# wglao/Adjoint-ODE-Adaptivity

Hardware: AMD Instinct MI355X
Metric: DOF-updates/sec, 1D DG advection fwd+adjoint sweep, N=4, K=1e6 (higher is better)
Workload: dtype f64

## Files before the change

### adjoint-ode-adaptivity_amd/csrc/dg_common.h

```cpp
#pragma once
#include <hip/hip_runtime.h>

#include <cmath>
#include <cstddef>
#include <cstdint>
#include <cstdio>
#include <cstdlib>
#include <cstring>
#include <initializer_list>
#include <new>
#include <string>
#include <tuple>
#include <vector>
#include <type_traits>
#include <utility>
#include <vector>

#include "dg_advec.h"
#include "dg_chain.h"
#include "dg_shape.h"

namespace dgk {

constexpr int kBlock = 256;
static_assert(kBlock == kTileLanes, "the shape rules (dg_shape.h) count tiles of kBlock lanes");
constexpr int kMaxNP = 9;
constexpr int kArgmaxParts = 1024;

#define DG_NL_STEP_ATTR __attribute__((amdgpu_num_sgpr(80)))
constexpr int kNLAdjMinWaves = 5;


__device__ __forceinline__ void eta_update(double* __restrict__ eta, int64_t e, double acc,
                                           int mode) {
  double v = (mode & kEtaAssign) ? acc : eta[e] + acc;
  if (mode & kEtaAbs) v = fabs(v);
  eta[e] = v;
}

__host__ __device__ constexpr int64_t rec_ld(int64_t ktot) { return (ktot + 1) & ~int64_t(1); }

template <class F> struct KernargLayout;
template <class... P> struct KernargLayout<void (*)(P...)> {
  static constexpr int kParams = int(sizeof...(P));
  using Tail = std::tuple_element_t<sizeof...(P) - 1, std::tuple<P...>>;
  static constexpr int kPointers = (0 + ... + int(std::is_pointer_v<P>));
  static constexpr size_t kTailOffset = size_t(kParams - 1) * sizeof(void*);
};

template <class F, class A>
__device__ __forceinline__ const char* kernarg_tail() {
  using L = KernargLayout<F>;
  static_assert(std::is_same_v<typename L::Tail, A>, "kernel's last parameter is not A");
  static_assert(L::kPointers == L::kParams - 1, "all parameters before A must be pointers");
  static_assert(sizeof(void*) == 8 && alignof(A) == 8, "A must follow 8-byte pointers unpadded");
  static_assert(std::is_standard_layout_v<A> && std::is_trivially_copyable_v<A>,
                "offsetof needs a standard-layout argument struct");
  return (const char*)__builtin_amdgcn_kernarg_segment_ptr() + L::kTailOffset;
}

#define DG_KAS __attribute__((address_space(4)))
template <class F, class A>
__device__ __forceinline__ const DG_KAS char* kernarg_tail_k() {
  (void)kernarg_tail<F, A>();
  return (const DG_KAS char*)__builtin_amdgcn_kernarg_segment_ptr() + KernargLayout<F>::kTailOffset;
}

constexpr size_t kKernargMax = 4096;

constexpr size_t kMarkBytes = 16384;

int fail(int code, const std::string& msg);

inline bool overlap(const void* x, size_t nx, const void* y, size_t ny) {
  const uintptr_t a = reinterpret_cast<uintptr_t>(x), b = reinterpret_cast<uintptr_t>(y);
  return a < b + ny && b < a + nx;
}

struct ArgRange {
  const char* name;
  const void* ptr;
  size_t bytes;
};

inline int disjoint(std::initializer_list<ArgRange> args) {
  for (const ArgRange* i = args.begin(); i != args.end(); ++i)
    for (const ArgRange* j = i + 1; j != args.end(); ++j)
      if (i->ptr && j->ptr && i->bytes && j->bytes && overlap(i->ptr, i->bytes, j->ptr, j->bytes))
        return fail(DG_ERR_ARG, std::string(i->name) + " and " + j->name +
                                    " overlap (the byte ranges of a call's arrays must be disjoint)");
  return DG_OK;
}

#define HIP_TRY(expr)                                                              \
  do {                                                                             \
    hipError_t e_ = (expr);                                                        \
    if (e_ != hipSuccess)                                                          \
      return ::dgk::fail(DG_ERR_HIP, std::string(#expr) + ": " + hipGetErrorString(e_));  \
  } while (0)

template <int NS> struct RK;
template <> struct RK<5> {
  __host__ __device__ static constexpr double A(int s) {
    return s == 0 ? 0.0
         : s == 1 ? -567301805773.0 / 1357537059087.0
         : s == 2 ? -2404267990393.0 / 2016746695238.0
         : s == 3 ? -3550918686646.0 / 2091501179385.0
                  : -1275806237668.0 / 842570457699.0;
  }
  __host__ __device__ static constexpr double B(int s) {
    return s == 0 ? 1432997174477.0 / 9575080441755.0
         : s == 1 ? 5161836677717.0 / 13612068292357.0
         : s == 2 ? 1720146321549.0 / 2090206949498.0
         : s == 3 ? 3134564353537.0 / 4481467310338.0
                  : 2277821191437.0 / 14882151754819.0;
  }
  __host__ __device__ static constexpr double C(int s) {
    return s == 0 ? 0.0
         : s == 1 ? 1432997174477.0 / 9575080441755.0
         : s == 2 ? 2526269341429.0 / 6820363962896.0
         : s == 3 ? 2006345519317.0 / 3224310063776.0
                  : 2802321613138.0 / 2924317926251.0;
  }
};
template <> struct RK<1> {
  __host__ __device__ static constexpr double A(int) { return 0.0; }
  __host__ __device__ static constexpr double B(int) { return 1.0; }
  __host__ __device__ static constexpr double C(int) { return 0.0; }
};

template <int NP> struct OpArgs {
  double Dm[NP * NP];
  double L0[NP];
  double L1[NP];
};

template <int NP> struct EOArgs {
  static constexpr int NE = (NP + 1) / 2;
  static constexpr int NO = NP / 2;
  double Qeo[NE * NO];
  double Qoe[NO * NE];
  double le[NE];
  double lo[NO];
};

template <int NP, int NS, int MS> struct StepArgs {
  EOArgs<NP> op;
  double sc;
  double uin[MS * NS + 1];
  int64_t ktot;
  int64_t stride;
  int64_t n0;
  int32_t K;
  int32_t xcd;
  int32_t jend;
};

template <int NP, int MS> struct AdjArgs {
  EOArgs<NP> op;
  double sc;
  double uin_res[MS];
  double src[MS];
  int64_t ktot;
  int64_t stride;
  int64_t n0;
  int32_t K;
  int32_t has_eta;
  int32_t xcd;
};

template <int NP>
__device__ __forceinline__ int load_tile(const double* __restrict__ g, int64_t e0, int64_t nd,
                                         double* __restrict__ lds) {
  const int64_t d0 = e0 * NP;
  const int64_t base = d0 & ~int64_t(1);
  const int off = int(d0 - base);
  const int nvec = (kBlock * NP + off + 1) >> 1;
  const double2* __restrict__ g2 = reinterpret_cast<const double2*>(g);
  for (int v = threadIdx.x; v < nvec; v += kBlock) {
    const int64_t gd = base + 2 * int64_t(v);
    double2 val;
    if (gd >= 0 && gd + 1 < nd) {
      val = g2[gd >> 1];
    } else {
      val.x = (gd >= 0 && gd < nd) ? g[gd] : 0.0;
      val.y = (gd + 1 >= 0 && gd + 1 < nd) ? g[gd + 1] : 0.0;
    }
    *reinterpret_cast<double2*>(&lds[2 * v]) = val;
  }
  return off;
}

template <int NP, int W> struct TileGeo {
  static constexpr int LB = kBlock * W;
  static constexpr int T = LB;
  static constexpr int kVec = (T * NP + 2 + 2 * LB - 1) / (2 * LB);
  static constexpr int kTileD = T * NP + 2;
  static constexpr int kFaceD = 4 * (T + 2);
  static constexpr int kFB = (kTileD + 1) & ~1;
  static constexpr int kLds = kFB + kFaceD;
};

template <int NP, int W> struct TileRegs {
  double2 v[TileGeo<NP, W>::kVec];
  int off;
};

template <int NP, int W, bool EDGE = true>
__device__ __forceinline__ void tile_issue(const double* __restrict__ g, int64_t e0, int64_t nd,
                                           TileRegs<NP, W>& r) {
  using G = TileGeo<NP, W>;
  const int64_t d0 = e0 * NP;
  const int64_t base = d0 & ~int64_t(1);
  r.off = int(d0 - base);
  const int nvec = (G::T * NP + r.off + 1) >> 1;
  const double2* __restrict__ g2 = reinterpret_cast<const double2*>(g);
#pragma unroll
  for (int q = 0; q < G::kVec; ++q) {
    const int v = threadIdx.x + q * G::LB;
    const int64_t gd = base + 2 * int64_t(v);
    double2 val = make_double2(0.0, 0.0);
    if (v < nvec) {
      if (!EDGE || (gd >= 0 && gd + 1 < nd)) {
        val = g2[gd >> 1];
      } else {
        if (gd >= 0 && gd < nd) val.x = g[gd];
        if (gd + 1 >= 0 && gd + 1 < nd) val.y = g[gd + 1];
      }
    }
    r.v[q] = val;
  }
}

template <int NP, int W>
__device__ __forceinline__ void tile_commit(const TileRegs<NP, W>& r, double* __restrict__ lds) {
  using G = TileGeo<NP, W>;
  const int nvec = (G::T * NP + r.off + 1) >> 1;
#pragma unroll
  for (int q = 0; q < G::kVec; ++q) {
    const int v = threadIdx.x + q * G::LB;
    if (v < nvec) *reinterpret_cast<double2*>(&lds[2 * v]) = r.v[q];
  }
}

template <int LB = kBlock>
__device__ __forceinline__ void store_run(double* __restrict__ g, int64_t o0, int64_t count,
                                          const double* __restrict__ lds) {
  double2* __restrict__ g2 = reinterpret_cast<double2*>(g);
  for (int64_t v = threadIdx.x; 2 * v < count; v += LB) {
    const double2 val = *reinterpret_cast<const double2*>(&lds[2 * v]);
    const int64_t gd = o0 + 2 * v;
    if (2 * v + 1 < count) {
      g2[gd >> 1] = val;
    } else {
      g[gd] = val.x;
    }
  }
}

template <int COUNT, int LB>
__device__ __forceinline__ void store_full(double* __restrict__ g, int64_t o0,
                                           const double* __restrict__ lds) {
  static_assert(COUNT % 2 == 0, "16-byte runs");
  constexpr int NV = COUNT / 2, NQ = (NV + LB - 1) / LB;
  double2* __restrict__ g2 = reinterpret_cast<double2*>(g + o0);
#pragma unroll
  for (int q = 0; q < NQ; ++q) {
    const int v = int(threadIdx.x) + q * LB;
    if ((q + 1) * LB <= NV || v < NV) g2[v] = *reinterpret_cast<const double2*>(&lds[2 * v]);
  }
}

__device__ __forceinline__ bool edge_tile(int64_t e0, int T, int64_t ktot, int32_t K) {
  if (e0 < 0 || e0 + T > ktot) return true;
  const int64_t kl0 = int64_t(uint32_t(e0) % uint32_t(K));
  return kl0 == 0 || kl0 + T >= K;
}

struct Elem {
  int64_t e;
  int32_t kl;
  bool inrange, first, last, valid;
};

template <int H, int T, bool EDGE = true>
__device__ __forceinline__ Elem elem_info(int64_t e0, int el, int64_t ktot, int32_t K) {
  Elem E;
  E.e = e0 + el;
  if constexpr (!EDGE) {
    E.kl = int32_t(uint32_t(E.e) % uint32_t(K));
    E.inrange = true;
    E.first = E.last = false;
    E.valid = el >= H && el < T - H;
    return E;
  }
  E.inrange = (E.e >= 0 && E.e < ktot);
  E.kl = E.inrange ? int32_t(uint32_t(E.e) % uint32_t(K)) : 0;
  E.first = (E.kl == 0);
  E.last = (E.kl == K - 1);
  E.valid = E.inrange && el >= H && el < T - H;
  return E;
}

__device__ __forceinline__ int64_t tile_of(int64_t b, int64_t n, bool xcd) {
  if (!xcd || n < 16) return b;
  const int64_t q = n / 8, r = n % 8, x = b % 8, j = b / 8;
  return (x < r ? x * (q + 1) : r * (q + 1) + (x - r) * q) + j;
}


__device__ __forceinline__ void pin(double& x) { asm volatile("" : "+v"(x)); }

template <int NP>
__device__ __forceinline__ void to_eo(const double* u, double* ev, double* od) {
  constexpr int NE = EOArgs<NP>::NE, NO = EOArgs<NP>::NO, N = NP - 1;
#pragma unroll
  for (int k = 0; k < NO; ++k) {
    ev[k] = 0.5 * (u[k] + u[N - k]);
    od[k] = 0.5 * (u[k] - u[N - k]);
  }
  if constexpr (NE > NO) ev[NO] = u[NO];
}

template <int NP>
__device__ __forceinline__ void from_eo(const double* ev, const double* od, double* u) {
  constexpr int NE = EOArgs<NP>::NE, NO = EOArgs<NP>::NO, N = NP - 1;
#pragma unroll
  for (int k = 0; k < NO; ++k) {
    u[k] = ev[k] + od[k];
    u[N - k] = ev[k] - od[k];
  }
  if constexpr (NE > NO) u[NO] = ev[NO];
}

template <int NP, int W, int H>
__device__ __forceinline__ void stage_out(double* __restrict__ lds, const double (*ev)[(NP + 1) / 2],
                                          const double (*od)[NP / 2], bool dual) {
  constexpr int T = TileGeo<NP, W>::T, EPL = 1;
  constexpr int NE = EOArgs<NP>::NE, NO = EOArgs<NP>::NO, N = NP - 1;
  const int lane = threadIdx.x;
#pragma unroll
  for (int m = 0; m < EPL; ++m) {
    const int el = m * T + lane;
    if (el >= H && el < T - H) {
      double* o = lds + (el - H) * NP;
      if (dual) {
#pragma unroll
        for (int k = 0; k < NO; ++k) {
          o[k] = 0.5 * (ev[m][k] + od[m][k]);
          o[N - k] = 0.5 * (ev[m][k] - od[m][k]);
        }
        if constexpr (NE > NO) o[NO] = ev[m][NO];
      } else {
        from_eo<NP>(ev[m], od[m], o);
      }
    }
  }
}

}

struct dg_plan : dgk::Shape {
  int N = 0;
  int64_t K = 0, batch = 0;
  int64_t K_cap = 0;
  double a = 0.0;
  int inflow = 0, scheme = 0;
  double s_uniform = 0.0;
  double r[dgk::kMaxNP], V[dgk::kMaxNP * dgk::kMaxNP], invV[dgk::kMaxNP * dgk::kMaxNP],
      Dr[dgk::kMaxNP * dgk::kMaxNP],
      LIFT[dgk::kMaxNP * 2];
  double* d_scale = nullptr;
  double* d_VX = nullptr;
  double* d_scratch = nullptr;
  double* d_scratch2 = nullptr;
  double* d_pv = nullptr;
  int64_t* d_pi = nullptr;
  void* d_mark = nullptr;
  void* d_sweep = nullptr;
  int32_t* d_nl_list = nullptr;
  int64_t nl_list_tiles = 0, nl_list_steps = 0;
  size_t sweep_bytes = 0;
  size_t sweep_sync = 0;
  int64_t sweep_items = -1;
  uint64_t sweep_sig = 0;
  std::vector<void*> sweep_retired;
  uint32_t* h_sweep_err = nullptr;
  uint32_t* d_sweep_err = nullptr;
  uint64_t* sweep_trace = nullptr;
  int cu_count = 0;
  int flux = 0;
  int limiter = 0;
  double tvb_M = 0.0;
  bool nonlinear() const { return flux != 0 || limiter != 0; }
};

namespace dgk {

inline double inflow_value(const dg_plan* p, double t) {
  if (p->inflow == DG_INFLOW_ZERO) return 0.0;
  return (p->inflow == DG_INFLOW_SIN_A2T) ? -std::sin(p->a * p->a * t) : -std::sin(p->a * t);
}

template <int NP> OpArgs<NP> make_op(const dg_plan* p, double scale = 1.0) {
  OpArgs<NP> op;
  for (int i = 0; i < NP; ++i) {
    for (int j = 0; j < NP; ++j) op.Dm[i * NP + j] = scale * (-p->a * p->Dr[i * NP + j]);
    op.L0[i] = scale * ((-p->a / 2.0) * p->LIFT[i * 2 + 0]);
    op.L1[i] = scale * ((p->a / 2.0) * p->LIFT[i * 2 + 1]);
  }
  return op;
}

template <int NP> bool make_eo(const dg_plan* p, double scale, EOArgs<NP>* out, bool fold = false) {
  constexpr int NE = EOArgs<NP>::NE, NO = EOArgs<NP>::NO, N = NP - 1;
  double Dm[NP][NP], L0[NP], L1[NP], T[NP][NP] = {}, Ti[NP][NP] = {};
  for (int i = 0; i < NP; ++i) {
    for (int j = 0; j < NP; ++j) Dm[i][j] = scale * (-p->a * p->Dr[i * NP + j]);
    L0[i] = scale * ((-p->a / 2.0) * p->LIFT[i * 2 + 0]);
    L1[i] = scale * ((p->a / 2.0) * p->LIFT[i * 2 + 1]);
  }
  for (int k = 0; k < NO; ++k) {
    T[k][k] += 0.5; T[k][N - k] += 0.5;
    T[NE + k][k] += 0.5; T[NE + k][N - k] -= 0.5;
    Ti[k][k] += 1.0; Ti[k][NE + k] += 1.0;
    Ti[N - k][k] += 1.0; Ti[N - k][NE + k] -= 1.0;
  }
  if (NE > NO) { T[NO][NO] = 1.0; Ti[NO][NO] = 1.0; }
  double TD[NP][NP], Q[NP][NP], l0[NP], l1[NP];
  for (int i = 0; i < NP; ++i)
    for (int j = 0; j < NP; ++j) {
      double t = 0.0;
      for (int k = 0; k < NP; ++k) t += T[i][k] * Dm[k][j];
      TD[i][j] = t;
    }
  double qmax = 0.0, lmax = 0.0;
  for (int i = 0; i < NP; ++i) {
    for (int j = 0; j < NP; ++j) {
      double t = 0.0;
      for (int k = 0; k < NP; ++k) t += TD[i][k] * Ti[k][j];
      Q[i][j] = t;
      qmax = std::fmax(qmax, std::fabs(t));
    }
    double a0 = 0.0, a1 = 0.0;
    for (int k = 0; k < NP; ++k) {
      a0 += T[i][k] * L0[k];
      a1 += T[i][k] * L1[k];
    }
    l0[i] = a0;
    l1[i] = a1;
    lmax = std::fmax(lmax, std::fmax(std::fabs(a0), std::fabs(a1)));
  }
  bool ok = true;
  const double tq = 1e-12 * qmax, tl = 1e-12 * lmax;
  for (int i = 0; i < NE; ++i)
    for (int j = 0; j < NE; ++j) ok = ok && std::fabs(Q[i][j]) <= tq;
  for (int i = 0; i < NO; ++i)
    for (int j = 0; j < NO; ++j) ok = ok && std::fabs(Q[NE + i][NE + j]) <= tq;
  for (int k = 0; k < NE; ++k) ok = ok && std::fabs(l0[k] + l1[k]) <= tl;
  for (int k = 0; k < NO; ++k) ok = ok && std::fabs(l0[NE + k] - l1[NE + k]) <= tl;
  if (out) {
    for (int k = 0; k < NE; ++k)
      for (int j = 0; j < NO; ++j) out->Qeo[k * NO + j] = Q[k][NE + j];
    for (int k = 0; k < NO; ++k)
      for (int j = 0; j < NE; ++j) out->Qoe[k * NE + j] = Q[NE + k][j];
    for (int k = 0; k < NE; ++k) out->le[k] = 0.5 * (l0[k] - l1[k]);
    for (int k = 0; k < NO; ++k) out->lo[k] = 0.5 * (l0[NE + k] + l1[NE + k]);
    if (fold) {
      for (int k = 0; k < NE; ++k) out->Qeo[k * NO] += 2.0 * out->le[k];
      for (int k = 0; k < NO; ++k) out->Qoe[k * NE] += 2.0 * out->lo[k];
    }
  }
  return ok;
}

template <int MAXNP = kMaxNP, class F> int dispatch_np(int np, F&& f) {
  static_assert(MAXNP >= 2 && MAXNP <= kMaxNP, "Np range");
  switch (np) {
    case 2: return f(std::integral_constant<int, 2>{});
    case 3: if constexpr (MAXNP >= 3) return f(std::integral_constant<int, 3>{}); break;
    case 4: if constexpr (MAXNP >= 4) return f(std::integral_constant<int, 4>{}); break;
    case 5: if constexpr (MAXNP >= 5) return f(std::integral_constant<int, 5>{}); break;
    case 6: if constexpr (MAXNP >= 6) return f(std::integral_constant<int, 6>{}); break;
    case 7: if constexpr (MAXNP >= 7) return f(std::integral_constant<int, 7>{}); break;
    case 8: if constexpr (MAXNP >= 8) return f(std::integral_constant<int, 8>{}); break;
    case 9: if constexpr (MAXNP >= 9) return f(std::integral_constant<int, 9>{}); break;
    default: break;
  }
  return fail(DG_ERR_ARG, "unsupported Np (2 .. " + std::to_string(MAXNP) + ")");
}
int nl_rhs(const dg_plan* p, const double* u, double* rhs, double t, hipStream_t st);
int nl_query(const dg_plan* p, int64_t out[3]);
int nl_fwd(dg_plan* p, double* u, double t0, double dt, int nsteps, double* snapshots,
           uint16_t* decisions, hipStream_t st);
int nl_adj(dg_plan* p, double* w, const double* snapshots, double t0, double dt, int nsteps,
           double src_coef, double* eta, int flags, const uint16_t* decisions, hipStream_t st);

int axpy_copy(const double* w, const double* u, double c, double* out, int64_t n, hipStream_t st);

inline auto field_copy(int64_t field, hipStream_t st) {
  return [=](double* dst, const double* src) -> int {
    HIP_TRY(hipMemcpyAsync(dst, src, sizeof(double) * field, hipMemcpyDeviceToDevice, st));
    return DG_OK;
  };
}

int fwd_march(const dg_plan* p, FwdShape s, double* u, const double* tn, double dt, int nsteps,
              double* snapshots, hipStream_t st);

int wave_launch_step(const dg_plan* p, int ms, const double* in, double* snap, double* last,
                     const double* times, double dt, hipStream_t st);

struct SweepBufs {
  double* U[9];
  double* W[9];
  double* rec;
  double* eta;
  double* part;
  uint32_t* sync;
  int64_t* am_idx;
  double* am_val;
  int64_t* am_nf;
  double* am_pv;
  int64_t* am_pi;
  uint32_t* err_host;
  int32_t spin_limit;
};
int sweep_waves_per_simd(const dg_plan* p, int waves);
int sweep_launch_rec(dg_plan* p, int waves, int msf, int msa, const SweepBufs& b, double t0,
                     double dt, int nsteps, int mode, hipStream_t st);
int sweep_sync_words();
int sweep_scratch(dg_plan* p, size_t sync_bytes, size_t data_bytes, hipStream_t st, char** data);
int sweep_watchdog(dg_plan* p);
int sweep_err_word();

int pair_launch_step_rec(const dg_plan* p, int ms, const double* in, double* rec, double* last,
                         const double* times, double dt, hipStream_t st, int64_t n0, bool jend);
int pair_launch_step_snap(const dg_plan* p, int ms, const double* in, double* snap,
                          const double* times, double dt, hipStream_t st);
int pair_launch_adj_rec(const dg_plan* p, int ms, const double* win, double* wout,
                        const double* rec, double* eta, int em, const double* t_next, double dt,
                        hipStream_t st, int64_t n0);

}
```

### adjoint-ode-adaptivity_amd/csrc/dg_ovl_tiles.h

```cpp
#pragma once
#include "dg_rec_tiles.h"

namespace dgr {

constexpr int kOvGL = kOvG / 2;

template <int NP, int NW> struct OvGeo {
  static constexpr int LB = 64 * NW;
  static constexpr int T = NW * kOvS + 2 * kOvG;
  static constexpr int kTileD = T * NP + 2;
  static constexpr int kVec = (kTileD + 2 * LB - 1) / (2 * LB);
  static constexpr int kXSlot = 2 * NP;
  static constexpr int kXBuf = NW * 2 * kOvGL * kXSlot;
  static constexpr int kXD = 2 * kXBuf;
  static constexpr int kLds = ((kTileD > kXD ? kTileD : kXD) + 1) & ~1;
  static_assert(kOvS % 2 == 0 && T % 2 == 0, "lane pairs at even elements");
};

__device__ __forceinline__ double ov_shr1(double x) {
  const long long b = __double_as_longlong(x);
  const int lo = int(b), hi = int(b >> 32);
  const int rl = __builtin_amdgcn_update_dpp(lo, lo, 0x138, 0xf, 0xf, false);
  const int rh = __builtin_amdgcn_update_dpp(hi, hi, 0x138, 0xf, 0xf, false);
  return __hiloint2double(rh, rl);
}
__device__ __forceinline__ double ov_shl1(double x) {
  const long long b = __double_as_longlong(x);
  const int lo = int(b), hi = int(b >> 32);
  const int rl = __builtin_amdgcn_update_dpp(lo, lo, 0x130, 0xf, 0xf, false);
  const int rh = __builtin_amdgcn_update_dpp(hi, hi, 0x130, 0xf, 0xf, false);
  return __hiloint2double(rh, rl);
}

struct OvLane {
  int wv, j, el0;
  bool own;
};
__device__ __forceinline__ OvLane ov_lane() {
  OvLane L;
  const int lane = threadIdx.x;
  L.wv = lane >> 6;
  L.j = lane & 63;
  L.el0 = L.wv * kOvS + 2 * L.j;
  L.own = L.j >= kOvGL && L.j < 64 - kOvGL;
  return L;
}

template <int NP, int NW>
__device__ __forceinline__ void ov_exchange(double* __restrict__ xb, const OvLane& L,
                                            double (*se)[(NP + 1) / 2], double (*so)[NP / 2]) {
  constexpr int NE = EOArgs<NP>::NE, NO = EOArgs<NP>::NO, SL = 2 * NP;
  static_assert(SL % 2 == 0, "16-byte slots");
  int slot = -1;
  if (L.j >= kOvGL && L.j < 2 * kOvGL) slot = (L.wv * 2 + 0) * kOvGL + (L.j - kOvGL);
  else if (L.j >= 64 - 2 * kOvGL && L.j < 64 - kOvGL)
    slot = (L.wv * 2 + 1) * kOvGL + (L.j - (64 - 2 * kOvGL));
  if (slot >= 0) {
    double v[SL];
#pragma unroll
    for (int m = 0; m < 2; ++m) {
#pragma unroll
      for (int k = 0; k < NE; ++k) v[m * NP + k] = se[m][k];
#pragma unroll
      for (int k = 0; k < NO; ++k) v[m * NP + NE + k] = so[m][k];
    }
    double2* p = reinterpret_cast<double2*>(xb + slot * SL);
#pragma unroll
    for (int q = 0; q < NP; ++q) p[q] = double2{v[2 * q], v[2 * q + 1]};
  }
  __syncthreads();
  int src = -1;
  if (L.j < kOvGL) {
    if (L.wv > 0) src = ((L.wv - 1) * 2 + 1) * kOvGL + L.j;
  } else if (L.j >= 64 - kOvGL) {
    if (L.wv < NW - 1) src = ((L.wv + 1) * 2 + 0) * kOvGL + (L.j - (64 - kOvGL));
  }
  if (src >= 0) {
    double v[SL];
    const double2* p = reinterpret_cast<const double2*>(xb + src * SL);
#pragma unroll
    for (int q = 0; q < NP; ++q) {
      const double2 t = p[q];
      v[2 * q] = t.x;
      v[2 * q + 1] = t.y;
    }
#pragma unroll
    for (int m = 0; m < 2; ++m) {
#pragma unroll
      for (int k = 0; k < NE; ++k) se[m][k] = v[m * NP + k];
#pragma unroll
      for (int k = 0; k < NO; ++k) so[m][k] = v[m * NP + NE + k];
    }
  }
}

template <int NP, int NW, int H, bool EDGE, bool WT>
__device__ __forceinline__ void ov_store(double* __restrict__ g, int64_t o0, int64_t nd,
                                         double* __restrict__ lds, const OvLane& L,
                                         const double (*ev)[(NP + 1) / 2],
                                         const double (*od)[NP / 2], bool dual) {
  using G = OvGeo<NP, NW>;
  constexpr int T = G::T, TE = T - 2 * H;
  constexpr int NE = EOArgs<NP>::NE, NO = EOArgs<NP>::NO, N = NP - 1;
  if (L.own) {
#pragma unroll
    for (int m = 0; m < 2; ++m) {
      const int el = L.el0 + m;
      if (el >= H && el < T - H) {
        double* o = lds + (el - H) * NP;
        if (dual) {
#pragma unroll
          for (int k = 0; k < NO; ++k) {
            o[k] = 0.5 * (ev[m][k] + od[m][k]);
            o[N - k] = 0.5 * (ev[m][k] - od[m][k]);
          }
          if constexpr (NE > NO) o[NO] = ev[m][NO];
        } else {
          from_eo<NP>(ev[m], od[m], o);
        }
      }
    }
  }
  __syncthreads();
  const int64_t rem = nd - o0;
  if constexpr (EDGE) {
    if constexpr (WT) store_run_wt<G::LB>(g, o0, rem < int64_t(TE) * NP ? rem : int64_t(TE) * NP, lds);
    else store_run<G::LB>(g, o0, rem < int64_t(TE) * NP ? rem : int64_t(TE) * NP, lds);
  } else {
    if constexpr (WT) store_full_wt<TE * NP, G::LB>(g, o0, lds);
    else store_full<TE * NP, G::LB>(g, o0, lds);
  }
}

template <int NP, bool UNI, int NW, int MS, bool EDGE, bool WT>
__device__ __forceinline__ void ov_step_tile(double* __restrict__ lds, int64_t tile,
                                             const double* __restrict__ uin,
                                             double* __restrict__ rec, double* __restrict__ last,
                                             const double* __restrict__ scale,
                                             const RpOp<NP>& c, OpSrc<NP> os,
                                             const double* kb, int64_t n0, bool jend) {
  using G = OvGeo<NP, NW>;
  constexpr int T = G::T, E = 2;
  constexpr int H = RpHalo<MS>::F;
  constexpr int TE = T - 2 * H;
  static_assert(TE % 2 == 0 && TE > 0 && H % 2 == 0 && H >= kOvG, "overlapped tiles");
  constexpr int NE = EOArgs<NP>::NE, NO = EOArgs<NP>::NO;
  constexpr int CB = G::kLds;
  constexpr int CR = CB + MS * 5;
  const int lane = threadIdx.x;
  const OvLane L = ov_lane();
  const int64_t e0 = tile * TE - H;
  const int64_t ec = e0 > 0 ? e0 : 0;
  const int64_t nd = c.ktot * NP;

  const int off = tile_load<G, NP, EDGE, WT>(uin, e0, nd, lds);
  if constexpr (EDGE) {
    if (lane <= MS * 6) lds[CB + lane] = kb[lane];
  }
  __syncthreads();
  double ue[E][NE], uo[E][NO];
  Elem El[E];
  double sc[E], jv[E];
#pragma unroll
  for (int m = 0; m < E; ++m) {
    const int el = L.el0 + m;
    const double* us = lds + off + el * NP;
    to_eo<NP>(us, ue[m], uo[m]);
    El[m] = elem_info<H, T, EDGE>(e0, el, c.ktot, c.K);
    El[m].valid = El[m].valid && L.own;
    sc[m] = c.sc;
    if constexpr (!UNI) sc[m] *= El[m].inrange ? scale[El[m].kl] : 0.0;
    jv[m] = us[0] - ((EDGE && El[m].first) ? lds[CR] : us[-1]);
  }
  if (n0 >= 1) rp_rec_put<E, EDGE, WT>(rec, n0 - 1, c.ktot, El, jv, ec);
  __syncthreads();

  const double b4 = c.beta[4], b5 = c.beta[5], b3 = c.beta[3], b2 = c.beta[2];
  double te[E][NE], to[E][NO];
#pragma unroll 1
  for (int st = 0; st < MS; ++st) {
#pragma unroll
    for (int l = 0; l < 5; ++l) {
      double v0[E], vN[E];
#pragma unroll
      for (int m = 0; m < E; ++m) {
        const double e = (l == 0) ? ue[m][0] : te[m][0], o = (l == 0) ? uo[m][0] : to[m][0];
        v0[m] = e + o;
        vN[m] = e - o;
      }
      const double fromL = ov_shr1(vN[E - 1]), fromR = ov_shl1(v0[0]);
      double pe[E][NE], po[E][NO];
      {
        const auto& op = os.get();
#pragma unroll
        for (int m = 0; m < E; ++m) {
#pragma unroll
          for (int k = 0; k < NE; ++k) {
            const double* vo = (l == 0) ? uo[m] : to[m];
            double a;
            int j0 = 0;
            if (UNI && l >= 3) {
              a = ue[m][k];
            } else if (UNI && l >= 1) {
              a = (l == 1 ? b3 : b2) * ue[m][k];
            } else {
              a = op.Qeo[k * NO] * vo[0];
              j0 = 1;
            }
#pragma unroll
            for (int j = j0; j < NO; ++j) a = fma(op.Qeo[k * NO + j], vo[j], a);
            pe[m][k] = a;
          }
#pragma unroll
          for (int k = 0; k < NO; ++k) {
            const double* ve = (l == 0) ? ue[m] : te[m];
            double a;
            int j0 = 0;
            if (UNI && l >= 3) {
              a = uo[m][k];
            } else if (UNI && l >= 1) {
              a = (l == 1 ? b3 : b2) * uo[m][k];
            } else {
              a = op.Qoe[k * NE] * ve[0];
              j0 = 1;
            }
#pragma unroll
            for (int j = j0; j < NE; ++j) a = fma(op.Qoe[k * NE + j], ve[j], a);
            po[m][k] = a;
          }
        }
      }
#pragma unroll
      for (int m = 0; m < E; ++m) {
#pragma unroll
        for (int k = 0; k < NE; ++k) pin(pe[m][k]);
#pragma unroll
        for (int k = 0; k < NO; ++k) pin(po[m][k]);
      }
      double bnd = 0.0, urec = 0.0;
      if constexpr (EDGE) {
        bnd = lds[CB + st * 5 + l];
        if (l == 0) urec = lds[CR + st];
      }
      const auto& ol = os.get();
#pragma unroll
      for (int m = 0; m < E; ++m) {
        double vL = (m == 0) ? fromL : vN[m - 1];
        double vR = (m == E - 1) ? fromR : v0[m + 1];
        if (l == 0) jv[m] = v0[m] - ((EDGE && El[m].first) ? urec : vL);
        if constexpr (EDGE) {
          vL = El[m].first ? bnd : vL;
          vR = El[m].last ? vN[m] : vR;
        }
        const double dlt = vR - vL, sig = -(vL + vR);
#pragma unroll
        for (int k = 0; k < NE; ++k) {
          const double z = fma(ol.le[k], dlt, pe[m][k]);
          if constexpr (UNI) {
            if (l == 0) te[m][k] = fma(b5, z, b4 * ue[m][k]);
            else if (l < 4) te[m][k] = z;
            else ue[m][k] = z;
          } else {
            if (l == 0) te[m][k] = fma(b5 * sc[m], z, b4 * ue[m][k]);
            else if (l < 3) te[m][k] = fma(sc[m], z, (l == 1 ? b3 : b2) * ue[m][k]);
            else if (l == 3) te[m][k] = fma(sc[m], z, ue[m][k]);
            else ue[m][k] = fma(sc[m], z, ue[m][k]);
          }
        }
#pragma unroll
        for (int k = 0; k < NO; ++k) {
          const double z = fma(ol.lo[k], sig, po[m][k]);
          if constexpr (UNI) {
            if (l == 0) to[m][k] = fma(b5, z, b4 * uo[m][k]);
            else if (l < 4) to[m][k] = z;
            else uo[m][k] = z;
          } else {
            if (l == 0) to[m][k] = fma(b5 * sc[m], z, b4 * uo[m][k]);
            else if (l < 3) to[m][k] = fma(sc[m], z, (l == 1 ? b3 : b2) * uo[m][k]);
            else if (l == 3) to[m][k] = fma(sc[m], z, uo[m][k]);
            else uo[m][k] = fma(sc[m], z, uo[m][k]);
          }
        }
      }
      if (l == 0 && st >= 1) rp_rec_put<E, EDGE, WT>(rec, n0 + st - 1, c.ktot, El, jv, ec);
    }
    if (st < MS - 1 || jend) ov_exchange<NP, NW>(lds + (st & 1) * G::kXBuf, L, ue, uo);
  }
  if (jend) {
    double u0[E], uN[E];
#pragma unroll
    for (int m = 0; m < E; ++m) {
      u0[m] = ue[m][0] + uo[m][0];
      uN[m] = ue[m][0] - uo[m][0];
    }
    const double fromL = ov_shr1(uN[E - 1]);
#pragma unroll
    for (int m = 0; m < E; ++m) {
      double uL = (m == 0) ? fromL : uN[m - 1];
      if constexpr (EDGE) uL = El[m].first ? lds[CR + MS] : uL;
      jv[m] = u0[m] - uL;
    }
    rp_rec_put<E, EDGE, WT>(rec, n0 + MS - 1, c.ktot, El, jv, ec);
  }
  __syncthreads();
  ov_store<NP, NW, H, EDGE, WT>(last, tile * TE * NP, nd, lds, L, ue, uo, false);
}

template <int NP, bool UNI, int NW, int MS, bool EDGE, bool WT>
__device__ __forceinline__ void ov_adj_tile(double* __restrict__ lds, int64_t tile,
                                            const double* __restrict__ win,
                                            double* __restrict__ wout,
                                            const double* __restrict__ rec,
                                            EtaSink& es,
                                            const double* __restrict__ scale,
                                            const RpOp<NP>& c, OpSrc<NP> os, int64_t n0) {
  using G = OvGeo<NP, NW>;
  constexpr int T = G::T, E = 2;
  constexpr int H = RpHalo<MS>::A;
  constexpr int TE = T - 2 * H;
  static_assert(TE % 2 == 0 && TE > 0 && H % 2 == 0 && H >= kOvG, "overlapped tiles");
  constexpr int NE = EOArgs<NP>::NE, NO = EOArgs<NP>::NO, N = NP - 1;
  const OvLane L = ov_lane();
  const int64_t e0 = tile * TE - H;
  const int64_t ec = e0 > 0 ? e0 : 0;
  const int64_t nd = c.ktot * NP;
  const int64_t ea = e0 + L.el0;
  const int has_eta = es.mode;

  const int off = tile_load<G, NP, EDGE, WT>(win, e0, nd, lds);
  double jn[E + 1];
  rp_rec_get<E, EDGE, WT>(rec, n0 + MS - 1, c.ktot, ea, ec, jn);
  __syncthreads();
  double we[E][NE], wo[E][NO];
  Elem El[E];
  double sc[E], eacc[E];
#pragma unroll
  for (int m = 0; m < E; ++m) {
    const int el = L.el0 + m;
    const double* w = lds + off + el * NP;
#pragma unroll
    for (int k = 0; k < NO; ++k) {
      we[m][k] = w[k] + w[N - k];
      wo[m][k] = w[k] - w[N - k];
    }
    if constexpr (NE > NO) we[m][NO] = w[NO];
    El[m] = elem_info<H, T, EDGE>(e0, el, c.ktot, c.K);
    El[m].valid = El[m].valid && L.own;
    sc[m] = c.sc;
    if constexpr (!UNI) sc[m] *= El[m].inrange ? scale[El[m].kl] : 0.0;
    eacc[m] = 0.0;
  }
  __syncthreads();

  const double b4 = c.beta[4], b5 = c.beta[5], b3 = c.beta[3], b2 = c.beta[2];
  double te[E][NE], to[E][NO];
#pragma unroll 1
  for (int st = MS - 1; st >= 0; --st) {
    double jc[E + 1];
#pragma unroll
    for (int m = 0; m <= E; ++m) jc[m] = jn[m];
    if (has_eta) {
      const auto& op = os.get();
#pragma unroll
      for (int m = 0; m < E; ++m) {
        double pe = 0.0, po = 0.0;
#pragma unroll
        for (int k = 0; k < NE; ++k) pe = fma(op.le[k], we[m][k], pe);
#pragma unroll
        for (int k = 0; k < NO; ++k) po = fma(op.lo[k], wo[m][k], po);
        const bool lst = EDGE && El[m].last;
        const double dd = lst ? jc[m] : jc[m] + jc[m + 1];
        const double ds = lst ? jc[m] : jc[m] - jc[m + 1];
        double cc = fma(dd, pe, ds * po);
        if constexpr (!UNI) cc *= sc[m];
        eacc[m] += cc;
      }
    }
    if (st > 0) rp_rec_get<E, EDGE, WT>(rec, n0 + st - 1, c.ktot, ea, ec, jn);
#pragma unroll
    for (int l = 0; l < 5; ++l) {
      double g0[E], g1[E], qe[E][NE], qo[E][NO];
      const auto& ol = os.get();
#pragma unroll
      for (int m = 0; m < E; ++m) {
        double gd = 0.0, gs = 0.0;
#pragma unroll
        for (int k = 0; k < NE; ++k) {
          const double v = (l == 0) ? we[m][k] : te[m][k];
          qe[m][k] = UNI ? v : sc[m] * v;
          gd = fma(ol.le[k], qe[m][k], gd);
        }
#pragma unroll
        for (int k = 0; k < NO; ++k) {
          const double v = (l == 0) ? wo[m][k] : to[m][k];
          qo[m][k] = UNI ? v : sc[m] * v;
          gs = fma(ol.lo[k], qo[m][k], gs);
        }
        g0[m] = gd + gs;
        g1[m] = gs - gd;
      }
      const double fromL = ov_shr1(g1[E - 1]), fromR = ov_shl1(g0[0]);
      double ae[E][NE], ao[E][NO];
      const auto& oq = os.get();
#pragma unroll
      for (int m = 0; m < E; ++m) {
#pragma unroll
        for (int j = 0; j < NO; ++j) {
          double t;
          int k0 = 0;
          if (l >= 3) {
            t = wo[m][j];
          } else if (l >= 1) {
            t = (l == 1 ? b3 : b2) * wo[m][j];
          } else {
            t = oq.Qeo[j] * qe[m][0];
            k0 = 1;
          }
#pragma unroll
          for (int k = k0; k < NE; ++k) t = fma(oq.Qeo[k * NO + j], qe[m][k], t);
          ao[m][j] = t;
        }
#pragma unroll
        for (int j = 0; j < NE; ++j) {
          double t;
          int k0 = 0;
          if (l >= 3) {
            t = we[m][j];
          } else if (l >= 1) {
            t = (l == 1 ? b3 : b2) * we[m][j];
          } else {
            t = oq.Qoe[j] * qo[m][0];
            k0 = 1;
          }
#pragma unroll
          for (int k = k0; k < NO; ++k) t = fma(oq.Qoe[k * NE + j], qo[m][k], t);
          ae[m][j] = t;
        }
#pragma unroll
        for (int k = 0; k < NO; ++k) pin(ao[m][k]);
#pragma unroll
        for (int k = 0; k < NE; ++k) pin(ae[m][k]);
      }
#pragma unroll
      for (int m = 0; m < E; ++m) {
        double gl = (m == 0) ? fromL : g1[m - 1];
        double gr = (m == E - 1) ? fromR : g0[m + 1];
        if constexpr (EDGE) {
          gl = El[m].first ? 0.0 : gl;
          gr = El[m].last ? g1[m] : gr;
        }
        ae[m][0] -= gl + gr;
        ao[m][0] += gr - gl;
#pragma unroll
        for (int k = 0; k < NE; ++k) {
          if (l == 0) te[m][k] = fma(b5, ae[m][k], b4 * we[m][k]);
          else if (l < 4) te[m][k] = ae[m][k];
          else we[m][k] = ae[m][k];
        }
#pragma unroll
        for (int k = 0; k < NO; ++k) {
          if (l == 0) to[m][k] = fma(b5, ao[m][k], b4 * wo[m][k]);
          else if (l < 4) to[m][k] = ao[m][k];
          else wo[m][k] = ao[m][k];
        }
      }
    }
    if (st > 0) ov_exchange<NP, NW>(lds + ((MS - 1 - st) & 1) * G::kXBuf, L, we, wo);
  }
  if (has_eta) {
    if constexpr (WT) {
      const __amdgpu_buffer_rsrc_t ro = wt_rsrc(es.part_out ? es.part_out + ec : es.eta + ec);
#pragma unroll
      for (int m = 0; m < E; ++m) {
        if (!El[m].valid) continue;
        const uint32_t o = uint32_t(El[m].e - ec) * 8u;
        if (es.part_out) {
          wt_st8(ro, o, eacc[m]);
        } else {
          double v;
          if (es.nparts > 0) {
            v = wt_ld8(wt_rsrc(es.part_in + ec), o);
            if (!(has_eta & kEtaAssign)) v = es.eta[El[m].e] + v;
            for (int q = 1; q < es.nparts; ++q)
              v = v + wt_ld8(wt_rsrc(es.part_in + q * es.part_ld + ec), o);
            v = v + eacc[m];
          } else {
            v = (has_eta & kEtaAssign) ? eacc[m] : es.eta[El[m].e] + eacc[m];
          }
          if (has_eta & kEtaAbs) v = fabs(v);
          wt_st8(ro, o, v);
          if (es.argmax && am_better(fabs(v), El[m].e, es.bv, es.bi)) {
            es.bv = fabs(v);
            es.bi = El[m].e;
          }
        }
      }
    } else {
#pragma unroll
      for (int m = 0; m < E; ++m)
        if (El[m].valid) eta_update(es.eta, El[m].e, eacc[m], has_eta);
    }
  }
  __syncthreads();
  ov_store<NP, NW, H, EDGE, WT>(wout, tile * TE * NP, nd, lds, L, we, wo, true);
}

}
```

### adjoint-ode-adaptivity_amd/csrc/dg_rec.hip

```cpp
#include "dg_rec_tiles.h"

namespace {
using namespace dgk;
using namespace dgr;

template <int NP, int MS> struct RpStepArgs {
  RpOp<NP> c;
  double bnd[MS * 5 + MS + 1];
  int64_t n0;
  int32_t jend;
};

template <int NP, int MS> struct RpAdjArgs {
  RpOp<NP> c;
  int64_t n0;
  int32_t has_eta;
};

template <int NP, bool UNI, int NW, int E, int MS>
__global__ __launch_bounds__(64 * NW) void k_step_rp(const double* __restrict__ uin,
                                                        double* __restrict__ rec,
                                                        double* __restrict__ last,
                                                        const double* __restrict__ scale,
                                                        RpStepArgs<NP, MS> args) {
  using G = RpGeo<NP, NW, E>;
  __shared__ __attribute__((aligned(16))) double lds[G::kLds + MS * 6 + 1];
  const int64_t tile = tile_of(blockIdx.x, gridDim.x, args.c.xcd);
  constexpr int H = RpHalo<MS>::F;
  const int64_t e0 = tile * (G::T - 2 * H) - H;
  using SArgs = RpStepArgs<NP, MS>;
  const OpSrc<NP> os = op_src<NP>(
      args.c, kernarg_tail_k<decltype(&k_step_rp<NP, UNI, NW, E, MS>), SArgs>() + offsetof(SArgs, c));
  if (edge_tile(e0, G::T, args.c.ktot, args.c.K)) {
    const double* kb = reinterpret_cast<const double*>(
        kernarg_tail<decltype(&k_step_rp<NP, UNI, NW, E, MS>), SArgs>() + offsetof(SArgs, bnd));
    rp_step_tile<NP, UNI, NW, E, MS, true, false>(lds, tile, uin, rec, last, scale, args.c, os,
                                                  kb, args.n0, args.jend);
  } else {
    rp_step_tile<NP, UNI, NW, E, MS, false, false>(lds, tile, uin, rec, last, scale, args.c, os,
                                                   nullptr, args.n0, args.jend);
  }
}

template <int NP, bool UNI, int NW, int E, int MS>
__global__ __launch_bounds__(64 * NW) void k_adj_rp(const double* __restrict__ win,
                                                       double* __restrict__ wout,
                                                       const double* __restrict__ rec,
                                                       double* __restrict__ eta,
                                                       const double* __restrict__ scale,
                                                       RpAdjArgs<NP, MS> args) {
  using G = RpGeo<NP, NW, E>;
  __shared__ __attribute__((aligned(16))) double lds[G::kLds];
  const int64_t tile = tile_of(blockIdx.x, gridDim.x, args.c.xcd);
  constexpr int H = RpHalo<MS>::A;
  const int64_t e0 = tile * (G::T - 2 * H) - H;
  EtaSink es{eta, nullptr, nullptr, 0, 0, args.has_eta, false, 0.0, 0};
  using AArgs = RpAdjArgs<NP, MS>;
  const OpSrc<NP> os = op_src<NP>(
      args.c, kernarg_tail_k<decltype(&k_adj_rp<NP, UNI, NW, E, MS>), AArgs>() + offsetof(AArgs, c));
  if (edge_tile(e0, G::T, args.c.ktot, args.c.K))
    rp_adj_tile<NP, UNI, NW, E, MS, true, false>(lds, tile, win, wout, rec, es, scale, args.c, os,
                                                 args.n0);
  else
    rp_adj_tile<NP, UNI, NW, E, MS, false, false>(lds, tile, win, wout, rec, es, scale, args.c,
                                                  os, args.n0);
}

template <int NP, bool UNI, int NW, int MS>
__global__ __launch_bounds__(64 * NW) void k_step_rps(const double* __restrict__ uin,
                                                         double* __restrict__ snap,
                                                         const double* __restrict__ scale,
                                                         RpStepArgs<NP, MS> args) {
  using G = RpGeo<NP, NW, 2>;
  __shared__ __attribute__((aligned(16))) double lds[G::kLds + MS * 6 + 1];
  const int64_t tile = tile_of(blockIdx.x, gridDim.x, args.c.xcd);
  constexpr int H = RpHalo<MS>::F;
  const int64_t e0 = tile * (G::T - 2 * H) - H;
  using SArgs = RpStepArgs<NP, MS>;
  const OpSrc<NP> os = op_src<NP>(
      args.c, kernarg_tail_k<decltype(&k_step_rps<NP, UNI, NW, MS>), SArgs>() + offsetof(SArgs, c));
  const int64_t field = args.c.ktot * NP;
  double* last = snap + (MS - 1) * field;
  if (edge_tile(e0, G::T, args.c.ktot, args.c.K)) {
    const double* kb = reinterpret_cast<const double*>(
        kernarg_tail<decltype(&k_step_rps<NP, UNI, NW, MS>), SArgs>() + offsetof(SArgs, bnd));
    rp_step_tile<NP, UNI, NW, 2, MS, true, false, true>(lds, tile, uin, snap, last, scale, args.c,
                                                        os, kb, 0, false, field);
  } else {
    rp_step_tile<NP, UNI, NW, 2, MS, false, false, true>(lds, tile, uin, snap, last, scale,
                                                         args.c, os, nullptr, 0, false, field);
  }
}

template <int NP, int NW, int MS>
int rp_snap_e(const dg_plan* p, const double* in, double* snap, const double* times, double dt,
              hipStream_t st) {
  RpStepArgs<NP, MS> a;
  if (const int rc = rp_make_op<NP>(p, dt, &a.c)) return rc;
  rp_block_bnd(p, MS, times, dt, a.bnd);
  a.n0 = 0;
  a.jend = 0;
  constexpr int TE = RpGeo<NP, NW, 2>::T - 2 * RpHalo<MS>::F;
  const unsigned grid = grid_for(p->ktot, TE);
  if (p->uniform)
    hipLaunchKernelGGL((k_step_rps<NP, true, NW, MS>), dim3(grid), dim3(64 * NW), 0, st, in, snap,
                       p->d_scale, a);
  else
    hipLaunchKernelGGL((k_step_rps<NP, false, NW, MS>), dim3(grid), dim3(64 * NW), 0, st, in,
                       snap, p->d_scale, a);
  HIP_TRY(hipGetLastError());
  return DG_OK;
}

template <int NP, int NW, int E, int MS>
int rp_step_e(const dg_plan* p, const double* in, double* rec, double* last, const double* times,
              double dt, hipStream_t st, int64_t n0, bool jend) {
  RpStepArgs<NP, MS> a;
  if (const int rc = rp_make_op<NP>(p, dt, &a.c)) return rc;
  rp_block_bnd(p, MS, times, dt, a.bnd);
  a.n0 = n0;
  a.jend = jend ? 1 : 0;
  constexpr int TE = RpGeo<NP, NW, E>::T - 2 * RpHalo<MS>::F;
  const unsigned grid = grid_for(p->ktot, TE);
  if (p->uniform)
    hipLaunchKernelGGL((k_step_rp<NP, true, NW, E, MS>), dim3(grid), dim3(64 * NW), 0, st, in,
                       rec, last, p->d_scale, a);
  else
    hipLaunchKernelGGL((k_step_rp<NP, false, NW, E, MS>), dim3(grid), dim3(64 * NW), 0, st, in,
                       rec, last, p->d_scale, a);
  HIP_TRY(hipGetLastError());
  return DG_OK;
}

template <int NP, int NW, int E, int MS>
int rp_adj_e(const dg_plan* p, const double* win, double* wout, const double* rec, double* eta,
             int eta_mode, const double* , double dt, hipStream_t st, int64_t n0) {
  RpAdjArgs<NP, MS> a;
  if (const int rc = rp_make_op<NP>(p, dt, &a.c)) return rc;
  a.n0 = n0;
  a.has_eta = eta != nullptr ? (eta_mode | kEtaOn) : 0;
  constexpr int TE = RpGeo<NP, NW, E>::T - 2 * RpHalo<MS>::A;
  const unsigned grid = grid_for(p->ktot, TE);
  if (p->uniform)
    hipLaunchKernelGGL((k_adj_rp<NP, true, NW, E, MS>), dim3(grid), dim3(64 * NW), 0, st, win,
                       wout, rec, eta, p->d_scale, a);
  else
    hipLaunchKernelGGL((k_adj_rp<NP, false, NW, E, MS>), dim3(grid), dim3(64 * NW), 0, st, win,
                       wout, rec, eta, p->d_scale, a);
  HIP_TRY(hipGetLastError());
  return DG_OK;
}

template <int N> using ic = std::integral_constant<int, N>;
template <int NW, bool REC, class F> int pair_steps(int ms, F&& f) {
  switch (ms) {
    case 20: if constexpr (REC && NW == 8) return f(ic<NW>{}, ic<20>{}); break;
    case 16: if constexpr (REC && NW == 8) return f(ic<NW>{}, ic<16>{}); break;
    case 10: if constexpr (REC) return f(ic<NW>{}, ic<10>{}); break;
    case 8: return f(ic<NW>{}, ic<8>{});
    case 5: if constexpr (REC) return f(ic<NW>{}, ic<5>{}); break;
    case 4: return f(ic<NW>{}, ic<4>{});
    case 2: return f(ic<NW>{}, ic<2>{});
    case 1: return f(ic<NW>{}, ic<1>{});
    default: break;
  }
  return fail(DG_ERR_ARG, "pair tiles: unsupported steps per launch for this tile width");
}
template <bool REC, class F> int pair_shape(int width, int ms, F&& f) {
  return width == 2 ? pair_steps<8, REC>(ms, f) : pair_steps<4, REC>(ms, f);
}

}

namespace dgk {

int pair_launch_step_rec(const dg_plan* p, int ms, const double* in, double* rec, double* last,
                         const double* times, double dt, hipStream_t st, int64_t n0, bool jend) {
  return dispatch_np(p->NP, [&](auto np) -> int {
    return pair_shape<true>(rec_fwd_width(p), ms, [&](auto nw, auto m) -> int {
      return rp_step_e<np, nw, 2, m>(p, in, rec, last, times, dt, st, n0, jend);
    });
  });
}

int pair_launch_step_snap(const dg_plan* p, int ms, const double* in, double* snap,
                          const double* times, double dt, hipStream_t st) {
  return dispatch_np(p->NP, [&](auto np) -> int {
    return pair_shape<false>(p->tile_width, ms, [&](auto nw, auto m) -> int {
      return rp_snap_e<np, nw, m>(p, in, snap, times, dt, st);
    });
  });
}

int pair_launch_adj_rec(const dg_plan* p, int ms, const double* win, double* wout,
                        const double* rec, double* eta, int em, const double* t_next, double dt,
                        hipStream_t st, int64_t n0) {
  return dispatch_np(p->NP, [&](auto np) -> int {
    return pair_shape<true>(p->rec_tile_width, ms, [&](auto nw, auto m) -> int {
      return rp_adj_e<np, nw, 2, m>(p, win, wout, rec, eta, em, t_next, dt, st, n0);
    });
  });
}

}
```

### adjoint-ode-adaptivity_amd/csrc/dg_rec_tiles.h

```cpp
#pragma once
#include "dg_common.h"

namespace dgr {
using namespace dgk;

template <int NP, int NW, int E> struct RpGeo {
  static constexpr int LB = 64 * NW;
  static constexpr int T = E * LB;
  static constexpr int kTileD = T * NP + 2;
  static constexpr int kVec = (kTileD + 2 * LB - 1) / (2 * LB);
  static constexpr int kFaceD = 4 * (LB + 2);
  static constexpr int kLds = ((kTileD > kFaceD ? kTileD : kFaceD) + 1) & ~1;
};

template <int MS> struct RpHalo {
  static constexpr int F = (MS * 5 + 2) & ~1;
  static constexpr int A = (MS * 5 + 1) & ~1;
};

typedef unsigned rp_v4u __attribute__((ext_vector_type(4)));
typedef unsigned rp_v2u __attribute__((ext_vector_type(2)));
constexpr int kSc1 = 16;

__device__ __forceinline__ __amdgpu_buffer_rsrc_t wt_rsrc(const void* base) {
  const uint64_t b = reinterpret_cast<uint64_t>(base);
  const uint32_t lo = __builtin_amdgcn_readfirstlane(uint32_t(b));
  const uint32_t hi = __builtin_amdgcn_readfirstlane(uint32_t(b >> 32));
  void* p = reinterpret_cast<void*>((uint64_t(hi) << 32) | lo);
  return __builtin_amdgcn_make_buffer_rsrc(p, 0, 0x7ffffff0, 0x00020000);
}
__device__ __forceinline__ void wt_st16(__amdgpu_buffer_rsrc_t r, uint32_t off, double2 v) {
  __builtin_amdgcn_raw_buffer_store_b128(__builtin_bit_cast(rp_v4u, v), r, off, 0, kSc1);
}
__device__ __forceinline__ void wt_st8(__amdgpu_buffer_rsrc_t r, uint32_t off, double v) {
  __builtin_amdgcn_raw_buffer_store_b64(__builtin_bit_cast(rp_v2u, v), r, off, 0, kSc1);
}
__device__ __forceinline__ double2 wt_ld16(__amdgpu_buffer_rsrc_t r, uint32_t off) {
  return __builtin_bit_cast(double2, __builtin_amdgcn_raw_buffer_load_b128(r, off, 0, kSc1));
}
__device__ __forceinline__ double wt_ld8(__amdgpu_buffer_rsrc_t r, uint32_t off) {
  return __builtin_bit_cast(double, __builtin_amdgcn_raw_buffer_load_b64(r, off, 0, kSc1));
}

template <class G, int NP, bool EDGE, bool WT>
__device__ __forceinline__ int tile_load(const double* __restrict__ g, int64_t e0, int64_t nd,
                                         double* __restrict__ lds) {
  const int64_t d0 = e0 * NP;
  const int64_t base = d0 & ~int64_t(1);
  const int off = int(d0 - base);
  const int nvec = (G::T * NP + off + 1) >> 1;
  const double2* __restrict__ g2 = reinterpret_cast<const double2*>(g);
  const int64_t bc = base > 0 ? base : 0;
  const __amdgpu_buffer_rsrc_t r = wt_rsrc(g + bc);
  double2 rv[G::kVec];
#pragma unroll
  for (int q = 0; q < G::kVec; ++q) {
    const int v = int(threadIdx.x) + q * G::LB;
    const int64_t gd = base + 2 * int64_t(v);
    double2 val = make_double2(0.0, 0.0);
    if (v < nvec) {
      if (!EDGE || (gd >= 0 && gd + 1 < nd)) {
        if constexpr (WT) val = wt_ld16(r, uint32_t(gd - bc) * 8u);
        else val = g2[gd >> 1];
      } else {
        if constexpr (WT) {
          if (gd >= 0 && gd < nd) val.x = wt_ld8(r, uint32_t(gd - bc) * 8u);
          if (gd + 1 >= 0 && gd + 1 < nd) val.y = wt_ld8(r, uint32_t(gd + 1 - bc) * 8u);
        } else {
          if (gd >= 0 && gd < nd) val.x = g[gd];
          if (gd + 1 >= 0 && gd + 1 < nd) val.y = g[gd + 1];
        }
      }
    }
    rv[q] = val;
  }
#pragma unroll
  for (int q = 0; q < G::kVec; ++q) {
    const int v = int(threadIdx.x) + q * G::LB;
    if (v < nvec) *reinterpret_cast<double2*>(&lds[2 * v]) = rv[q];
  }
  return off;
}

template <int NP, int NW, int E, bool EDGE, bool WT>
__device__ __forceinline__ int rp_load(const double* __restrict__ g, int64_t e0, int64_t nd,
                                       double* __restrict__ lds) {
  return tile_load<RpGeo<NP, NW, E>, NP, EDGE, WT>(g, e0, nd, lds);
}

template <int LB>
__device__ __forceinline__ void store_run_wt(double* __restrict__ g, int64_t o0, int64_t count,
                                             const double* __restrict__ lds) {
  const __amdgpu_buffer_rsrc_t r = wt_rsrc(g + o0);
  for (int64_t v = threadIdx.x; 2 * v < count; v += LB) {
    const double2 val = *reinterpret_cast<const double2*>(&lds[2 * v]);
    if (2 * v + 1 < count) wt_st16(r, uint32_t(v) * 16u, val);
    else wt_st8(r, uint32_t(v) * 16u, val.x);
  }
}

template <int COUNT, int LB>
__device__ __forceinline__ void store_full_wt(double* __restrict__ g, int64_t o0,
                                              const double* __restrict__ lds) {
  static_assert(COUNT % 2 == 0, "16-byte runs");
  constexpr int NV = COUNT / 2, NQ = (NV + LB - 1) / LB;
  const __amdgpu_buffer_rsrc_t r = wt_rsrc(g + o0);
#pragma unroll
  for (int q = 0; q < NQ; ++q) {
    const int v = int(threadIdx.x) + q * LB;
    if ((q + 1) * LB <= NV || v < NV)
      wt_st16(r, uint32_t(v) * 16u, *reinterpret_cast<const double2*>(&lds[2 * v]));
  }
}

template <int NP, int NW, int E, int H, bool EDGE, bool WT>
__device__ __forceinline__ void rp_store(double* __restrict__ g, int64_t o0, int64_t nd,
                                         double* __restrict__ lds,
                                         const double (*ev)[(NP + 1) / 2],
                                         const double (*od)[NP / 2], bool dual) {
  using G = RpGeo<NP, NW, E>;
  constexpr int T = G::T, TE = T - 2 * H;
  constexpr int NE = EOArgs<NP>::NE, NO = EOArgs<NP>::NO, N = NP - 1;
  const int lane = threadIdx.x;
#pragma unroll
  for (int m = 0; m < E; ++m) {
    const int el = E * lane + m;
    if (el >= H && el < T - H) {
      double* o = lds + (el - H) * NP;
      if (dual) {
#pragma unroll
        for (int k = 0; k < NO; ++k) {
          o[k] = 0.5 * (ev[m][k] + od[m][k]);
          o[N - k] = 0.5 * (ev[m][k] - od[m][k]);
        }
        if constexpr (NE > NO) o[NO] = ev[m][NO];
      } else {
        from_eo<NP>(ev[m], od[m], o);
      }
    }
  }
  __syncthreads();
  const int64_t rem = nd - o0;
  if constexpr (EDGE) {
    if constexpr (WT) store_run_wt<G::LB>(g, o0, rem < int64_t(TE) * NP ? rem : int64_t(TE) * NP, lds);
    else store_run<G::LB>(g, o0, rem < int64_t(TE) * NP ? rem : int64_t(TE) * NP, lds);
  } else {
    if constexpr (WT) store_full_wt<TE * NP, G::LB>(g, o0, lds);
    else store_full<TE * NP, G::LB>(g, o0, lds);
  }
}

template <int E, bool EDGE, bool WT>
__device__ __forceinline__ void rp_rec_put(double* __restrict__ rec, int64_t n, int64_t ktot,
                                           const Elem* El, const double* jv, int64_t ec) {
  double* row = rec + n * rec_ld(ktot);
  if constexpr (WT) {
    const __amdgpu_buffer_rsrc_t r = wt_rsrc(row + ec);
    const uint32_t o = uint32_t(El[0].e - ec) * 8u;
#pragma unroll
    for (int q = 0; q < E; q += 2) {
      if (!EDGE || (El[q].valid && El[q + 1].valid)) {
        if (El[q].valid) wt_st16(r, o + 8u * q, double2{jv[q], jv[q + 1]});
      } else {
        if (El[q].valid) wt_st8(r, o + 8u * q, jv[q]);
        if (El[q + 1].valid) wt_st8(r, o + 8u * (q + 1), jv[q + 1]);
      }
    }
  } else {
#pragma unroll
    for (int q = 0; q < E; q += 2) {
      if (!EDGE || (El[q].valid && El[q + 1].valid)) {
        if (El[q].valid) *reinterpret_cast<double2*>(row + El[q].e) = double2{jv[q], jv[q + 1]};
      } else {
        if (El[q].valid) row[El[q].e] = jv[q];
        if (El[q + 1].valid) row[El[q + 1].e] = jv[q + 1];
      }
    }
  }
}

template <int E, bool EDGE, bool WT>
__device__ __forceinline__ void rp_rec_get(const double* __restrict__ rec, int64_t n,
                                           int64_t ktot, int64_t ea, int64_t ec, double* j) {
  const double* row = rec + n * rec_ld(ktot);
  if constexpr (WT) {
    const __amdgpu_buffer_rsrc_t r = wt_rsrc(row + ec);
    const uint32_t o = uint32_t(ea - ec) * 8u;
    if constexpr (!EDGE) {
#pragma unroll
      for (int q = 0; q < E; q += 2) {
        const double2 v = wt_ld16(r, o + 8u * q);
        j[q] = v.x;
        j[q + 1] = v.y;
      }
      j[E] = wt_ld8(r, o + 8u * E);
    } else {
#pragma unroll
      for (int m = 0; m <= E; ++m) j[m] = (ea + m >= 0 && ea + m < ktot) ? wt_ld8(r, o + 8u * m) : 0.0;
    }
  } else {
    if constexpr (!EDGE) {
#pragma unroll
      for (int q = 0; q < E; q += 2) {
        const double2 v = *reinterpret_cast<const double2*>(row + ea + q);
        j[q] = v.x;
        j[q + 1] = v.y;
      }
      j[E] = row[ea + E];
    } else {
#pragma unroll
      for (int m = 0; m <= E; ++m) j[m] = (ea + m >= 0 && ea + m < ktot) ? row[ea + m] : 0.0;
    }
  }
}

struct RkPoly {
  double beta[6];
  double g[5][5];
  bool ok;
};

inline const RkPoly& rk_poly() {
  static const RkPoly P = [] {
    long double uc[6] = {1}, rc[6] = {0}, uf[5][6] = {}, rf[5][6] = {};
    for (int s = 0; s < 5; ++s) {
      const long double A = RK<5>::A(s), B = RK<5>::B(s);
      for (int k = 5; k >= 0; --k) rc[k] = A * rc[k] + (k ? uc[k - 1] : 0.0L);
      for (int q = 0; q < 5; ++q)
        for (int k = 5; k >= 0; --k)
          rf[q][k] = A * rf[q][k] + (k ? uf[q][k - 1] : 0.0L) + ((q == s && k == 0) ? 1.0L : 0.0L);
      for (int k = 0; k < 6; ++k) uc[k] += B * rc[k];
      for (int q = 0; q < 5; ++q)
        for (int k = 0; k < 6; ++k) uf[q][k] += B * rf[q][k];
    }
    RkPoly r{};
    for (int k = 0; k < 6; ++k) r.beta[k] = double(uc[k]);
    for (int q = 0; q < 5; ++q)
      for (int k = 0; k < 5; ++k) r.g[q][k] = double(uf[q][k]);
    r.ok = r.beta[0] == 1.0 && r.beta[1] == 1.0 && r.beta[5] != 0.0;
    return r;
  }();
  return P;
}

inline void rp_block_bnd(const dg_plan* p, int MS, const double* times, double dt, double* bnd) {
  const RkPoly& P = rk_poly();
  for (int m = 0; m < MS; ++m) {
    double u[5], b[5];
    for (int s = 0; s < 5; ++s) u[s] = inflow_value(p, times[m] + RK<5>::C(s) * dt);
    for (int k = 0; k < 5; ++k) {
      double acc = 0.0;
      for (int s = 0; s < 5; ++s) acc = std::fma(P.g[s][k], u[s], acc);
      b[k] = acc;
    }
    bnd[m * 5 + 0] = b[4] / P.beta[5];
    for (int l = 1; l < 5; ++l) bnd[m * 5 + l] = b[4 - l];
  }
  for (int m = 0; m <= MS; ++m) bnd[MS * 5 + m] = inflow_value(p, times[m]);
}

template <int NP> struct RpOp {
  EOArgs<NP> op;
  double sc;
  double beta[6];
  int64_t ktot;
  int32_t K;
  int32_t xcd;
};

template <int NP> int rp_make_op(const dg_plan* p, double dt, RpOp<NP>* c) {
  const RkPoly& P = rk_poly();
  if (!P.ok) return fail(DG_ERR_HIP, "LSERK4 stability polynomial: beta_0 = beta_1 = 1 expected");
  make_eo<NP>(p, p->uniform ? dt * p->s_uniform : 1.0, &c->op, true);
  c->sc = dt;
  for (int k = 0; k < 6; ++k) c->beta[k] = P.beta[k];
  c->ktot = p->ktot;
  c->K = int32_t(p->K);
  c->xcd = p->xcd_order;
  return DG_OK;
}

template <int NP> constexpr bool kOpReload = NP >= 6;
template <int NP, bool R = kOpReload<NP>> struct OpSrc {
  const EOArgs<NP>* p;
  __device__ __forceinline__ const EOArgs<NP>& get() const { return *p; }
};
template <int NP> struct OpSrc<NP, true> {
  const DG_KAS EOArgs<NP>* p;
  __device__ __forceinline__ const DG_KAS EOArgs<NP>& get() const {
    const DG_KAS EOArgs<NP>* q = p;
    asm volatile("" : "+s"(q));
    return *q;
  }
};
template <int NP>
__device__ __forceinline__ OpSrc<NP> op_src(const RpOp<NP>& rc, const DG_KAS char* kc) {
  if constexpr (kOpReload<NP>)
    return OpSrc<NP>{reinterpret_cast<const DG_KAS EOArgs<NP>*>(kc + offsetof(RpOp<NP>, op))};
  else
    return OpSrc<NP>{&rc.op};
}

template <int NP, int E, bool EDGE>
__device__ __forceinline__ void rp_snap_put(double* __restrict__ g, const Elem* El,
                                            const double (*ue)[(NP + 1) / 2],
                                            const double (*uo)[NP / 2]) {
  double v[E][NP];
#pragma unroll
  for (int m = 0; m < E; ++m) from_eo<NP>(ue[m], uo[m], v[m]);
  const bool pair = El[0].valid && El[1].valid;
  double* o = g + El[0].e * NP;
  if (pair && (reinterpret_cast<uintptr_t>(o) & 15) == 0) {
#pragma unroll
    for (int q = 0; q < NP; ++q)
      reinterpret_cast<double2*>(o)[q] = double2{v[(2 * q) / NP][(2 * q) % NP],
                                                 v[(2 * q + 1) / NP][(2 * q + 1) % NP]};
  } else {
#pragma unroll
    for (int m = 0; m < E; ++m)
      if (El[m].valid) {
#pragma unroll
        for (int i = 0; i < NP; ++i) g[El[m].e * NP + i] = v[m][i];
      }
  }
}

template <int NP, bool UNI, int NW, int E, int MS, bool EDGE, bool WT, bool SNAP = false>
__device__ __forceinline__ void rp_step_tile(double* __restrict__ lds, int64_t tile,
                                             const double* __restrict__ uin,
                                             double* __restrict__ rec, double* __restrict__ last,
                                             const double* __restrict__ scale,
                                             const RpOp<NP>& c, OpSrc<NP> os,
                                             const double* kb, int64_t n0, bool jend,
                                             int64_t sstride = 0) {
  static_assert(!SNAP || (E == 2 && !WT), "snapshots: launch chains on pair tiles");
  using G = RpGeo<NP, NW, E>;
  constexpr int T = G::T, LB = G::LB;
  constexpr int H = RpHalo<MS>::F;
  constexpr int TE = T - 2 * H;
  static_assert(TE % 2 == 0 && TE > 0 && H % 2 == 0 && (E == 2 || E == 4),
                "pair tiles: aligned pairs");
  constexpr int NE = EOArgs<NP>::NE, NO = EOArgs<NP>::NO;
  constexpr int CB = G::kLds;
  constexpr int CR = CB + MS * 5;
  constexpr int FB = LB + 2;
  const int lane = threadIdx.x;
  const int64_t e0 = tile * TE - H;
  const int64_t ec = e0 > 0 ? e0 : 0;
  const int64_t nd = c.ktot * NP;

  const int off = rp_load<NP, NW, E, EDGE, WT>(uin, e0, nd, lds);
  if constexpr (EDGE) {
    if (lane <= MS * 6) lds[CB + lane] = kb[lane];
  }
  __syncthreads();
  double ue[E][NE], uo[E][NO];
  Elem El[E];
  double sc[E], jv[E];
#pragma unroll
  for (int m = 0; m < E; ++m) {
    const int el = E * lane + m;
    const double* us = lds + off + el * NP;
    to_eo<NP>(us, ue[m], uo[m]);
    El[m] = elem_info<H, T, EDGE>(e0, el, c.ktot, c.K);
    sc[m] = c.sc;
    if constexpr (!UNI) sc[m] *= El[m].inrange ? scale[El[m].kl] : 0.0;
    jv[m] = us[0] - ((EDGE && El[m].first) ? lds[CR] : us[-1]);
  }
  if constexpr (!SNAP)
    if (n0 >= 1) rp_rec_put<E, EDGE, WT>(rec, n0 - 1, c.ktot, El, jv, ec);
  __syncthreads();

  const double b4 = c.beta[4], b5 = c.beta[5], b3 = c.beta[3], b2 = c.beta[2];
  double te[E][NE], to[E][NO];
#pragma unroll 1
  for (int st = 0; st < MS; ++st) {
#pragma unroll
    for (int l = 0; l < 5; ++l) {
      const int fL = ((st * 5 + l) & 1) * 2 * FB;
      const int fR = fL + FB;
      double v0[E], vN[E];
#pragma unroll
      for (int m = 0; m < E; ++m) {
        const double e = (l == 0) ? ue[m][0] : te[m][0], o = (l == 0) ? uo[m][0] : to[m][0];
        v0[m] = e + o;
        vN[m] = e - o;
      }
      lds[fL + lane + 1] = v0[0];
      lds[fR + lane + 1] = vN[E - 1];
      __builtin_amdgcn_sched_barrier(0);
      double pe[E][NE], po[E][NO];
      {
        const auto& op = os.get();
#pragma unroll
        for (int m = 0; m < E; ++m) {
#pragma unroll
          for (int k = 0; k < NE; ++k) {
            const double* vo = (l == 0) ? uo[m] : to[m];
            double a;
            int j0 = 0;
            if (UNI && l >= 3) {
              a = ue[m][k];
            } else if (UNI && l >= 1) {
              a = (l == 1 ? b3 : b2) * ue[m][k];
            } else {
              a = op.Qeo[k * NO] * vo[0];
              j0 = 1;
            }
#pragma unroll
            for (int j = j0; j < NO; ++j) a = fma(op.Qeo[k * NO + j], vo[j], a);
            pe[m][k] = a;
          }
        }
      }
      {
        const auto& op = os.get();
#pragma unroll
        for (int m = 0; m < E; ++m) {
#pragma unroll
          for (int k = 0; k < NO; ++k) {
            const double* ve = (l == 0) ? ue[m] : te[m];
            double a;
            int j0 = 0;
            if (UNI && l >= 3) {
              a = uo[m][k];
            } else if (UNI && l >= 1) {
              a = (l == 1 ? b3 : b2) * uo[m][k];
            } else {
              a = op.Qoe[k * NE] * ve[0];
              j0 = 1;
            }
#pragma unroll
            for (int j = j0; j < NE; ++j) a = fma(op.Qoe[k * NE + j], ve[j], a);
            po[m][k] = a;
          }
        }
      }
#pragma unroll
      for (int m = 0; m < E; ++m) {
#pragma unroll
        for (int k = 0; k < NE; ++k) pin(pe[m][k]);
#pragma unroll
        for (int k = 0; k < NO; ++k) pin(po[m][k]);
      }
      __syncthreads();
      const double fromL = lds[fR + lane], fromR = lds[fL + lane + 2];
      double bnd = 0.0, urec = 0.0;
      if constexpr (EDGE) {
        bnd = lds[CB + st * 5 + l];
        if (l == 0) urec = lds[CR + st];
      }
      const auto& ol = os.get();
#pragma unroll
      for (int m = 0; m < E; ++m) {
        double vL = (m == 0) ? fromL : vN[m - 1];
        double vR = (m == E - 1) ? fromR : v0[m + 1];
        if (l == 0) jv[m] = v0[m] - ((EDGE && El[m].first) ? urec : vL);
        if constexpr (EDGE) {
          vL = El[m].first ? bnd : vL;
          vR = El[m].last ? vN[m] : vR;
        }
        const double dlt = vR - vL, sig = -(vL + vR);
#pragma unroll
        for (int k = 0; k < NE; ++k) {
          const double z = fma(ol.le[k], dlt, pe[m][k]);
          if constexpr (UNI) {
            if (l == 0) te[m][k] = fma(b5, z, b4 * ue[m][k]);
            else if (l < 4) te[m][k] = z;
            else ue[m][k] = z;
          } else {
            if (l == 0) te[m][k] = fma(b5 * sc[m], z, b4 * ue[m][k]);
            else if (l < 3) te[m][k] = fma(sc[m], z, (l == 1 ? b3 : b2) * ue[m][k]);
            else if (l == 3) te[m][k] = fma(sc[m], z, ue[m][k]);
            else ue[m][k] = fma(sc[m], z, ue[m][k]);
          }
        }
#pragma unroll
        for (int k = 0; k < NO; ++k) {
          const double z = fma(ol.lo[k], sig, po[m][k]);
          if constexpr (UNI) {
            if (l == 0) to[m][k] = fma(b5, z, b4 * uo[m][k]);
            else if (l < 4) to[m][k] = z;
            else uo[m][k] = z;
          } else {
            if (l == 0) to[m][k] = fma(b5 * sc[m], z, b4 * uo[m][k]);
            else if (l < 3) to[m][k] = fma(sc[m], z, (l == 1 ? b3 : b2) * uo[m][k]);
            else if (l == 3) to[m][k] = fma(sc[m], z, uo[m][k]);
            else uo[m][k] = fma(sc[m], z, uo[m][k]);
          }
        }
      }
      if constexpr (!SNAP)
        if (l == 0 && st >= 1) rp_rec_put<E, EDGE, WT>(rec, n0 + st - 1, c.ktot, El, jv, ec);
    }
    if constexpr (SNAP)
      if (st < MS - 1) rp_snap_put<NP, E, EDGE>(rec + st * sstride, El, ue, uo);
  }
  if (!SNAP && jend) {
    const int fL = ((MS * 5) & 1) * 2 * FB, fR = fL + FB;
    double u0[E], uN[E];
#pragma unroll
    for (int m = 0; m < E; ++m) {
      u0[m] = ue[m][0] + uo[m][0];
      uN[m] = ue[m][0] - uo[m][0];
    }
    lds[fL + lane + 1] = u0[0];
    lds[fR + lane + 1] = uN[E - 1];
    __syncthreads();
    const double fromL = lds[fR + lane];
#pragma unroll
    for (int m = 0; m < E; ++m) {
      double uL = (m == 0) ? fromL : uN[m - 1];
      if constexpr (EDGE) uL = El[m].first ? lds[CR + MS] : uL;
      jv[m] = u0[m] - uL;
    }
    rp_rec_put<E, EDGE, WT>(rec, n0 + MS - 1, c.ktot, El, jv, ec);
  }
  __syncthreads();
  rp_store<NP, NW, E, H, EDGE, WT>(last, tile * TE * NP, nd, lds, ue, uo, false);
}

struct EtaSink {
  double* eta;
  double* part_out;
  const double* part_in;
  int64_t part_ld;
  int32_t nparts;
  int32_t mode;
  bool argmax;
  double bv;
  int64_t bi;
};

__device__ __forceinline__ bool am_better(double va, int64_t ia, double vb, int64_t ib) {
  const bool na = isnan(va), nb = isnan(vb);
  if (na != nb) return na;
  if (!na && va != vb) return va > vb;
  return ia < ib;
}

template <int NP, bool UNI, int NW, int E, int MS, bool EDGE, bool WT>
__device__ __forceinline__ void rp_adj_tile(double* __restrict__ lds, int64_t tile,
                                            const double* __restrict__ win,
                                            double* __restrict__ wout,
                                            const double* __restrict__ rec,
                                            EtaSink& es,
                                            const double* __restrict__ scale,
                                            const RpOp<NP>& c, OpSrc<NP> os, int64_t n0) {
  using G = RpGeo<NP, NW, E>;
  constexpr int T = G::T, LB = G::LB;
  constexpr int H = RpHalo<MS>::A;
  constexpr int TE = T - 2 * H;
  static_assert(TE % 2 == 0 && TE > 0 && H % 2 == 0 && (E == 2 || E == 4),
                "pair tiles: aligned pairs");
  constexpr int NE = EOArgs<NP>::NE, NO = EOArgs<NP>::NO, N = NP - 1;
  constexpr int FB = LB + 2;
  const int lane = threadIdx.x;
  const int64_t e0 = tile * TE - H;
  const int64_t ec = e0 > 0 ? e0 : 0;
  const int64_t nd = c.ktot * NP;
  const int64_t ea = e0 + E * lane;
  const int has_eta = es.mode;

  const int off = rp_load<NP, NW, E, EDGE, WT>(win, e0, nd, lds);
  double jn[E + 1];
  rp_rec_get<E, EDGE, WT>(rec, n0 + MS - 1, c.ktot, ea, ec, jn);
  __syncthreads();
  double we[E][NE], wo[E][NO];
  Elem El[E];
  double sc[E], eacc[E];
#pragma unroll
  for (int m = 0; m < E; ++m) {
    const int el = E * lane + m;
    const double* w = lds + off + el * NP;
#pragma unroll
    for (int k = 0; k < NO; ++k) {
      we[m][k] = w[k] + w[N - k];
      wo[m][k] = w[k] - w[N - k];
    }
    if constexpr (NE > NO) we[m][NO] = w[NO];
    El[m] = elem_info<H, T, EDGE>(e0, el, c.ktot, c.K);
    sc[m] = c.sc;
    if constexpr (!UNI) sc[m] *= El[m].inrange ? scale[El[m].kl] : 0.0;
    eacc[m] = 0.0;
  }
  __syncthreads();

  const double b4 = c.beta[4], b5 = c.beta[5], b3 = c.beta[3], b2 = c.beta[2];
  double te[E][NE], to[E][NO];
#pragma unroll 1
  for (int st = MS - 1; st >= 0; --st) {
    double jc[E + 1];
#pragma unroll
    for (int m = 0; m <= E; ++m) jc[m] = jn[m];
    if (has_eta) {
      const auto& op = os.get();
#pragma unroll
      for (int m = 0; m < E; ++m) {
        double pe = 0.0, po = 0.0;
#pragma unroll
        for (int k = 0; k < NE; ++k) pe = fma(op.le[k], we[m][k], pe);
#pragma unroll
        for (int k = 0; k < NO; ++k) po = fma(op.lo[k], wo[m][k], po);
        const bool lst = EDGE && El[m].last;
        const double dd = lst ? jc[m] : jc[m] + jc[m + 1];
        const double ds = lst ? jc[m] : jc[m] - jc[m + 1];
        double cc = fma(dd, pe, ds * po);
        if constexpr (!UNI) cc *= sc[m];
        eacc[m] += cc;
      }
    }
    if (st > 0) rp_rec_get<E, EDGE, WT>(rec, n0 + st - 1, c.ktot, ea, ec, jn);
#pragma unroll
    for (int l = 0; l < 5; ++l) {
      const int f0 = (((MS - 1 - st) * 5 + l) & 1) * 2 * FB, f1 = f0 + FB;
      double g0[E], g1[E], qe[E][NE], qo[E][NO];
      const auto& ol = os.get();
#pragma unroll
      for (int m = 0; m < E; ++m) {
        double gd = 0.0, gs = 0.0;
#pragma unroll
        for (int k = 0; k < NE; ++k) {
          const double v = (l == 0) ? we[m][k] : te[m][k];
          qe[m][k] = UNI ? v : sc[m] * v;
          gd = fma(ol.le[k], qe[m][k], gd);
        }
#pragma unroll
        for (int k = 0; k < NO; ++k) {
          const double v = (l == 0) ? wo[m][k] : to[m][k];
          qo[m][k] = UNI ? v : sc[m] * v;
          gs = fma(ol.lo[k], qo[m][k], gs);
        }
        g0[m] = gd + gs;
        g1[m] = gs - gd;
      }
      lds[f0 + lane + 1] = g0[0];
      lds[f1 + lane + 1] = g1[E - 1];
      __builtin_amdgcn_sched_barrier(0);
      double ae[E][NE], ao[E][NO];
      const auto& oq = os.get();
#pragma unroll
      for (int m = 0; m < E; ++m) {
#pragma unroll
        for (int j = 0; j < NO; ++j) {
          double t;
          int k0 = 0;
          if (l >= 3) {
            t = wo[m][j];
          } else if (l >= 1) {
            t = (l == 1 ? b3 : b2) * wo[m][j];
          } else {
            t = oq.Qeo[j] * qe[m][0];
            k0 = 1;
          }
#pragma unroll
          for (int k = k0; k < NE; ++k) t = fma(oq.Qeo[k * NO + j], qe[m][k], t);
          ao[m][j] = t;
        }
#pragma unroll
        for (int k = 0; k < NO; ++k) pin(ao[m][k]);
      }
      __builtin_amdgcn_sched_barrier(0);
      const auto& or_ = os.get();
#pragma unroll
      for (int m = 0; m < E; ++m) {
#pragma unroll
        for (int j = 0; j < NE; ++j) {
          double t;
          int k0 = 0;
          if (l >= 3) {
            t = we[m][j];
          } else if (l >= 1) {
            t = (l == 1 ? b3 : b2) * we[m][j];
          } else {
            t = or_.Qoe[j] * qo[m][0];
            k0 = 1;
          }
#pragma unroll
          for (int k = k0; k < NO; ++k) t = fma(or_.Qoe[k * NE + j], qo[m][k], t);
          ae[m][j] = t;
        }
#pragma unroll
        for (int k = 0; k < NE; ++k) pin(ae[m][k]);
      }
      __syncthreads();
      const double fromL = lds[f1 + lane], fromR = lds[f0 + lane + 2];
#pragma unroll
      for (int m = 0; m < E; ++m) {
        double gl = (m == 0) ? fromL : g1[m - 1];
        double gr = (m == E - 1) ? fromR : g0[m + 1];
        if constexpr (EDGE) {
          gl = El[m].first ? 0.0 : gl;
          gr = El[m].last ? g1[m] : gr;
        }
        ae[m][0] -= gl + gr;
        ao[m][0] += gr - gl;
#pragma unroll
        for (int k = 0; k < NE; ++k) {
          if (l == 0) te[m][k] = fma(b5, ae[m][k], b4 * we[m][k]);
          else if (l < 4) te[m][k] = ae[m][k];
          else we[m][k] = ae[m][k];
        }
#pragma unroll
        for (int k = 0; k < NO; ++k) {
          if (l == 0) to[m][k] = fma(b5, ao[m][k], b4 * wo[m][k]);
          else if (l < 4) to[m][k] = ao[m][k];
          else wo[m][k] = ao[m][k];
        }
      }
    }
  }
  if (has_eta) {
    if constexpr (WT) {
      const __amdgpu_buffer_rsrc_t ro = wt_rsrc(es.part_out ? es.part_out + ec : es.eta + ec);
#pragma unroll
      for (int m = 0; m < E; ++m) {
        if (!El[m].valid) continue;
        const uint32_t o = uint32_t(El[m].e - ec) * 8u;
        if (es.part_out) {
          wt_st8(ro, o, eacc[m]);
        } else {
          double v;
          if (es.nparts > 0) {
            v = wt_ld8(wt_rsrc(es.part_in + ec), o);
            if (!(has_eta & kEtaAssign)) v = es.eta[El[m].e] + v;
            for (int q = 1; q < es.nparts; ++q)
              v = v + wt_ld8(wt_rsrc(es.part_in + q * es.part_ld + ec), o);
            v = v + eacc[m];
          } else {
            v = (has_eta & kEtaAssign) ? eacc[m] : es.eta[El[m].e] + eacc[m];
          }
          if (has_eta & kEtaAbs) v = fabs(v);
          wt_st8(ro, o, v);
          if (es.argmax && am_better(fabs(v), El[m].e, es.bv, es.bi)) {
            es.bv = fabs(v);
            es.bi = El[m].e;
          }
        }
      }
    } else {
#pragma unroll
      for (int m = 0; m < E; ++m)
        if (El[m].valid) eta_update(es.eta, El[m].e, eacc[m], has_eta);
    }
  }
  __syncthreads();
  rp_store<NP, NW, E, H, EDGE, WT>(wout, tile * TE * NP, nd, lds, we, wo, true);
}

}
```

### adjoint-ode-adaptivity_amd/csrc/dg_sweep_kernel.h

```cpp
#pragma once
#include "dg_ovl_tiles.h"
#include "dg_flow.h"

namespace {
using namespace dgk;
using namespace dgr;

template <int NP, int MSF> struct SweepArgs {
  RpOp<NP> c;
  double bnd[(kSweepMaxSteps / MSF) * (MSF * 6 + 1)];
  double* U[kSweepMaxBlocks + 1];
  double* W[kSweepMaxBlocks + 1];
  double* rec;
  double* eta;
  double* part;
  const double* scale;
  uint32_t* sync;
  uint64_t* trace;
  int64_t* am_idx;
  double* am_val;
  int64_t* am_nf;
  double* am_pv;
  int64_t* am_pi;
  uint32_t* err_host;
  int32_t nbF, nbA, nTF, nTA;
  int32_t nsteps;
  int32_t mode;
  int32_t spin_limit;
};

template <int NP, bool UNI, int NW = 8, int X = 0> struct SweepOcc {
  static constexpr int waves_per_simd =
      (UNI && NP == 2 && (NW == 4 || NW == 8 || (X == 1 && NW == 16))) ? 8
      : (UNI && NP <= 5)                                               ? 6
                                                                       : 1;
};

template <int NP, int NW, int E, int X>
using SwGeo = std::conditional_t<X == 1, OvGeo<NP, NW>, RpGeo<NP, NW, E>>;

template <int NP, bool UNI, int NW, int MSF, int MSA, int E, int X>
__global__ __launch_bounds__(64 * NW) __attribute__((amdgpu_waves_per_eu(
    E == 2 ? SweepOcc<NP, UNI, NW, X>::waves_per_simd : 1))) void k_sweep_rp(SweepArgs<NP, MSF> a) {
  static_assert(X == 0 || E == 2, "overlapped waves hold element pairs");
  static_assert(sizeof(SweepArgs<NP, MSF>) <= kKernargMax,
                "k_sweep_rp's arguments exceed the kernarg segment");
  using G = SwGeo<NP, NW, E, X>;
  constexpr int HF = RpHalo<MSF>::F, HA = RpHalo<MSA>::A;
  constexpr int TEF = G::T - 2 * HF, TEA = G::T - 2 * HA;
  __shared__ __attribute__((aligned(16))) double lds[G::kLds + MSF * 6 + 1];
  __shared__ uint32_t s_item, s_epoch, s_last, s_bad;
  __shared__ double s_av[NW];
  __shared__ int64_t s_ai[NW];
  uint32_t* sync = a.sync;
  uint32_t* flags = sync + kSyncFlags;
  const int tid = threadIdx.x;
  const int64_t ktot = a.c.ktot;
  const int nTF = a.nTF, nTA = a.nTA, nbF = a.nbF, nbA = a.nbA;
  const int64_t nF = int64_t(nbF) * nTF;
  const int64_t nItems = nF + int64_t(nbA) * nTA;
  if (tid == 0) {
    uint32_t it, ep;
    flow_take(sync, nItems, &it, &ep);
    s_epoch = ep;
    s_item = it;
    s_bad = 0u;
  }
  __syncthreads();
  const int64_t item = s_item;
  const uint32_t epoch = s_epoch;
  const uint64_t t_deq = a.trace ? uint64_t(wall_clock64()) : 0;
  {
    const bool fwd = item < nF;
    int blk, j;
    int64_t d0 = 0;
    int nd = 0;
    if (fwd) {
      blk = int(item / nTF);
      j = int(item - int64_t(blk) * nTF);
      if (blk > 0) {
        const int lo = j > 0 ? j - 1 : 0, hi = j + 1 < nTF ? j + 1 : nTF - 1;
        d0 = int64_t(blk - 1) * nTF + lo;
        nd = hi - lo + 1;
      }
    } else {
      const int64_t i2 = item - nF;
      blk = int(i2 / nTA);
      j = int(i2 - int64_t(blk) * nTA);
      if (blk == 0) {
        int64_t elo = int64_t(j) * TEA - HA, ehi = int64_t(j + 1) * TEA + HA;
        elo = elo > 0 ? elo : 0;
        ehi = ehi < ktot - 1 ? ehi : ktot - 1;
        const int lo = int(elo / TEF), hi = int(ehi / TEF);
        d0 = int64_t(nbF - 1) * nTF + lo;
        nd = hi - lo + 1;
      } else {
        const int lo = j > 0 ? j - 1 : 0, hi = j + 1 < nTA ? j + 1 : nTA - 1;
        d0 = nF + int64_t(blk - 1) * nTA + lo;
        nd = hi - lo + 1;
      }
    }
    if (tid < 64 && nd > 0) {
      const bool gave_up = sweep_wait(flags + d0, nd, epoch, sync, a.err_host, a.spin_limit);
      if (tid == 0 && gave_up) s_bad = 1u;
    }
    __builtin_amdgcn_fence(__ATOMIC_ACQUIRE, "wavefront");
    __syncthreads();
    const uint64_t t_ready = a.trace ? uint64_t(wall_clock64()) : 0;
    using SA = SweepArgs<NP, MSF>;
    const DG_KAS char* ka = kernarg_tail_k<decltype(&k_sweep_rp<NP, UNI, NW, MSF, MSA, E, X>), SA>();
    const OpSrc<NP> os = op_src<NP>(a.c, ka + offsetof(SA, c));
    if (fwd) {
      const int64_t e0 = int64_t(j) * TEF - HF;
      const double* kb = reinterpret_cast<const double*>(
                             kernarg_tail<decltype(&k_sweep_rp<NP, UNI, NW, MSF, MSA, E, X>), SA>() +
                             offsetof(SA, bnd)) + blk * (MSF * 6 + 1);
      const int64_t n0 = int64_t(blk) * MSF;
      const bool jend = blk == a.nbF - 1;
      if constexpr (X == 1) {
        if (edge_tile(e0, G::T, ktot, a.c.K))
          ov_step_tile<NP, UNI, NW, MSF, true, true>(lds, j, a.U[blk], a.rec, a.U[blk + 1],
                                                     a.scale, a.c, os, kb, n0, jend);
        else
          ov_step_tile<NP, UNI, NW, MSF, false, true>(lds, j, a.U[blk], a.rec, a.U[blk + 1],
                                                      a.scale, a.c, os, kb, n0, jend);
      } else {
        if (edge_tile(e0, G::T, ktot, a.c.K))
          rp_step_tile<NP, UNI, NW, E, MSF, true, true>(lds, j, a.U[blk], a.rec, a.U[blk + 1],
                                                        a.scale, a.c, os, kb, n0, jend);
        else
          rp_step_tile<NP, UNI, NW, E, MSF, false, true>(lds, j, a.U[blk], a.rec, a.U[blk + 1],
                                                         a.scale, a.c, os, kb, n0, jend);
      }
      if (s_bad) {
        asm volatile("s_waitcnt vmcnt(0)" ::: "memory");
        __syncthreads();
        const int64_t o0 = int64_t(j) * TEF * NP, nd = ktot * NP;
        poison_run<64 * NW>(a.U[blk + 1], o0, (nd - o0) < int64_t(TEF) * NP ? nd - o0
                                                                            : int64_t(TEF) * NP);
        const int64_t ee = int64_t(j) * TEF, ne = (ktot - ee) < TEF ? ktot - ee : int64_t(TEF);
        const int64_t n0 = int64_t(blk) * MSF, r0 = n0 >= 1 ? n0 - 1 : 0;
        const int64_t r1 = (blk == a.nbF - 1) ? n0 + MSF : n0 + MSF - 1;
        for (int64_t r = r0; r < r1; ++r) poison_run<64 * NW>(a.rec + r * rec_ld(ktot), ee, ne);
      }
    } else {
      const int64_t e0 = int64_t(j) * TEA - HA;
      const bool lastb = blk == a.nbA - 1;
      EtaSink es;
      es.eta = a.eta;
      es.part_out = (a.mode && !lastb) ? a.part + int64_t(blk) * ktot : nullptr;
      es.part_in = a.part;
      es.part_ld = ktot;
      es.nparts = lastb ? a.nbA - 1 : 0;
      es.mode = a.mode;
      es.argmax = lastb && a.am_idx != nullptr;
      es.bv = -INFINITY;
      es.bi = INT64_MAX;
      const int64_t n0 = int64_t(a.nsteps) - int64_t(blk + 1) * MSA;
      if constexpr (X == 1) {
        if (edge_tile(e0, G::T, ktot, a.c.K))
          ov_adj_tile<NP, UNI, NW, MSA, true, true>(lds, j, a.W[blk], a.W[blk + 1], a.rec, es,
                                                    a.scale, a.c, os, n0);
        else
          ov_adj_tile<NP, UNI, NW, MSA, false, true>(lds, j, a.W[blk], a.W[blk + 1], a.rec, es,
                                                     a.scale, a.c, os, n0);
      } else {
        if (edge_tile(e0, G::T, ktot, a.c.K))
          rp_adj_tile<NP, UNI, NW, E, MSA, true, true>(lds, j, a.W[blk], a.W[blk + 1], a.rec, es,
                                                       a.scale, a.c, os, n0);
        else
          rp_adj_tile<NP, UNI, NW, E, MSA, false, true>(lds, j, a.W[blk], a.W[blk + 1], a.rec,
                                                        es, a.scale, a.c, os, n0);
      }
      if (s_bad) {
        asm volatile("s_waitcnt vmcnt(0)" ::: "memory");
        __syncthreads();
        const int64_t o0 = int64_t(j) * TEA, nd = ktot * NP;
        const int64_t ne = (ktot - o0) < TEA ? ktot - o0 : int64_t(TEA);
        poison_run<64 * NW>(a.W[blk + 1], o0 * NP, (nd - o0 * NP) < int64_t(TEA) * NP
                                                       ? nd - o0 * NP : int64_t(TEA) * NP);
        if (a.mode) poison_run<64 * NW>(es.part_out ? es.part_out : a.eta, o0, ne);
        es.bv = __builtin_nan("");
      }
      if (es.argmax) {
        wg_argmax<NW>(es.bv, es.bi, s_av, s_ai);
        if (tid == 0) {
          st8_agent(a.am_pv + j, __builtin_bit_cast(uint64_t, es.bv));
          st8_agent(a.am_pi + j, uint64_t(es.bi));
        }
      }
    }
    asm volatile("s_waitcnt vmcnt(0)" ::: "memory");
    __syncthreads();
    if (tid == 0) st_agent(flags + item, epoch);
    if (!fwd && blk == nbA - 1 && a.am_idx != nullptr) {
      flow_refine_arrive<NW>(sync, nTA, a.am_pv, a.am_pi, a.am_idx, a.am_val, a.am_nf, &s_last,
                             s_av, s_ai);
    }
    if (a.trace && tid == 0) {
      uint32_t xcc;
      asm volatile("s_getreg_b32 %0, hwreg(HW_REG_XCC_ID)" : "=s"(xcc));
      uint64_t* tr = a.trace + 4 * item;
      tr[0] = t_deq;
      tr[1] = t_ready;
      tr[2] = uint64_t(wall_clock64());
      tr[3] = (uint64_t(xcc) << 32) | blockIdx.x;
    }
  }
}

static_assert(kSweepMaxBlocks + 1 == sizeof(SweepBufs::U) / sizeof(double*), "SweepBufs");

template <int NP, bool UNI, int NW, int MSF, int MSA, int E, int X>
int sweep_launch(dg_plan* p, const dgk::SweepBufs& b, double t0, double dt, int nsteps,
                 int mode, hipStream_t st) {
  SweepArgs<NP, MSF> a;
  if (const int rc = rp_make_op<NP>(p, dt, &a.c)) return rc;
  const int nbF = nsteps / MSF, nbA = nsteps / MSA;
  const std::vector<double> tn = dgk::chain::time_levels(t0, dt, nsteps);
  for (int bk = 0; bk < nbF; ++bk)
    rp_block_bnd(p, MSF, &tn[size_t(bk) * MSF], dt, a.bnd + bk * (MSF * 6 + 1));
  for (int i = 0; i <= kSweepMaxBlocks; ++i) {
    a.U[i] = b.U[i];
    a.W[i] = b.W[i];
  }
  a.rec = b.rec;
  a.eta = b.eta;
  a.part = b.part;
  a.scale = p->d_scale;
  a.sync = b.sync;
  a.trace = p->sweep_trace;
  a.am_idx = b.am_idx;
  a.am_val = b.am_val;
  a.am_nf = b.am_nf;
  a.am_pv = b.am_pv;
  a.am_pi = b.am_pi;
  a.nbF = nbF;
  a.nbA = nbA;
  using G = SwGeo<NP, NW, E, X>;
  a.nTF = int(grid_for(p->ktot, G::T - 2 * RpHalo<MSF>::F));
  a.nTA = int(grid_for(p->ktot, G::T - 2 * RpHalo<MSA>::A));
  a.nsteps = nsteps;
  a.mode = mode;
  a.err_host = b.err_host;
  a.spin_limit = b.spin_limit > 0 ? b.spin_limit : kSweepSpinLimit;
  const int64_t items = int64_t(nbF) * a.nTF + int64_t(nbA) * a.nTA;
  hipLaunchKernelGGL((k_sweep_rp<NP, UNI, NW, MSF, MSA, E, X>), dim3(unsigned(items)), dim3(64 * NW), 0,
                     st, a);
  HIP_TRY(hipGetLastError());
  return DG_OK;
}

template <int NP, bool UNI, int NW, int E, int X>
int sweep_shape_launch(dg_plan* p, int msf, int msa, const dgk::SweepBufs& b, double t0,
                       double dt, int nsteps, int mode, hipStream_t st) {
  if constexpr (NW > 8 || X == 1) {
    if (msa == 10 && msf == 20) return sweep_launch<NP, UNI, NW, 20, 10, E, X>(p, b, t0, dt, nsteps, mode, st);
    if (msa == 10 && msf == 10) return sweep_launch<NP, UNI, NW, 10, 10, E, X>(p, b, t0, dt, nsteps, mode, st);
    return fail(DG_ERR_ARG, "dataflow sweep: 12 or 16 waves, or overlapped waves, take 10- or "
                            "20-step forward and 10-step adjoint blocks");
  } else {
    if (msa == 10) {
      if constexpr (NW * E >= 16)
        if (msf == 20) return sweep_launch<NP, UNI, NW, 20, 10, E, 0>(p, b, t0, dt, nsteps, mode, st);
      if (msf == 10) return sweep_launch<NP, UNI, NW, 10, 10, E, 0>(p, b, t0, dt, nsteps, mode, st);
      if (msf == 5) return sweep_launch<NP, UNI, NW, 5, 10, E, 0>(p, b, t0, dt, nsteps, mode, st);
    } else if (msa == 5) {
      if constexpr (NW * E >= 16)
        if (msf == 20) return sweep_launch<NP, UNI, NW, 20, 5, E, 0>(p, b, t0, dt, nsteps, mode, st);
      if (msf == 10) return sweep_launch<NP, UNI, NW, 10, 5, E, 0>(p, b, t0, dt, nsteps, mode, st);
      if (msf == 5) return sweep_launch<NP, UNI, NW, 5, 5, E, 0>(p, b, t0, dt, nsteps, mode, st);
    }
    return fail(DG_ERR_ARG, "dataflow sweep: unsupported steps per block for this tile width");
  }
}

template <int NP, int NW, int E = 2, int X = 0>
int sweep_uni(dg_plan* p, int msf, int msa, const dgk::SweepBufs& b, double t0, double dt,
              int nsteps, int mode, hipStream_t st) {
  return p->uniform
             ? sweep_shape_launch<NP, true, NW, E, X>(p, msf, msa, b, t0, dt, nsteps, mode, st)
             : sweep_shape_launch<NP, false, NW, E, X>(p, msf, msa, b, t0, dt, nsteps, mode, st);
}

}
```

Measured before the change: 812.8 billion.

## Fold LSERK stability-polynomial coefficients into per-level scaled operators for adjoint

Rewrites the adjoint's polynomial (Horner) evaluation of the five-stage RK step. Instead of multiplying by beta ratios each level, it precomputes four operator copies pre-scaled by the ratios on the host. For uniform meshes with NP other than 3 and at most 8, the adjoint tile then skips the per-level beta scaling multiplies and the final fma combine. This trades larger kernel arguments (five operator blocks) and forced operator reloads from the kernarg segment for fewer FP64 multiplies per level, with slightly different rounding.

```diff
diff --git a/adjoint-ode-adaptivity_amd/csrc/dg_common.h b/adjoint-ode-adaptivity_amd/csrc/dg_common.h
--- a/adjoint-ode-adaptivity_amd/csrc/dg_common.h
+++ b/adjoint-ode-adaptivity_amd/csrc/dg_common.h
@@ -18,6 +18,7 @@
 
 #include "dg_advec.h"
 #include "dg_chain.h"
+#include "dg_horner.h"
 #include "dg_shape.h"
 
 namespace dgk {
@@ -66,7 +67,6 @@
   return (const DG_KAS char*)__builtin_amdgcn_kernarg_segment_ptr() + KernargLayout<F>::kTailOffset;
 }
 
-constexpr size_t kKernargMax = 4096;
 
 constexpr size_t kMarkBytes = 16384;
 
@@ -99,35 +99,6 @@
       return ::dgk::fail(DG_ERR_HIP, std::string(#expr) + ": " + hipGetErrorString(e_));  \
   } while (0)
 
-template <int NS> struct RK;
-template <> struct RK<5> {
-  __host__ __device__ static constexpr double A(int s) {
-    return s == 0 ? 0.0
-         : s == 1 ? -567301805773.0 / 1357537059087.0
-         : s == 2 ? -2404267990393.0 / 2016746695238.0
-         : s == 3 ? -3550918686646.0 / 2091501179385.0
-                  : -1275806237668.0 / 842570457699.0;
-  }
-  __host__ __device__ static constexpr double B(int s) {
-    return s == 0 ? 1432997174477.0 / 9575080441755.0
-         : s == 1 ? 5161836677717.0 / 13612068292357.0
-         : s == 2 ? 1720146321549.0 / 2090206949498.0
-         : s == 3 ? 3134564353537.0 / 4481467310338.0
-                  : 2277821191437.0 / 14882151754819.0;
-  }
-  __host__ __device__ static constexpr double C(int s) {
-    return s == 0 ? 0.0
-         : s == 1 ? 1432997174477.0 / 9575080441755.0
-         : s == 2 ? 2526269341429.0 / 6820363962896.0
-         : s == 3 ? 2006345519317.0 / 3224310063776.0
-                  : 2802321613138.0 / 2924317926251.0;
-  }
-};
-template <> struct RK<1> {
-  __host__ __device__ static constexpr double A(int) { return 0.0; }
-  __host__ __device__ static constexpr double B(int) { return 1.0; }
-  __host__ __device__ static constexpr double C(int) { return 0.0; }
-};
 
 template <int NP> struct OpArgs {
   double Dm[NP * NP];
diff --git a/adjoint-ode-adaptivity_amd/csrc/dg_horner.h b/adjoint-ode-adaptivity_amd/csrc/dg_horner.h
--- /dev/null
+++ b/adjoint-ode-adaptivity_amd/csrc/dg_horner.h
@@ -0,0 +1,116 @@
+#pragma once
+#include <cmath>
+#include <cstddef>
+#include <cstdint>
+
+#include "dg_shape.h"
+
+#if defined(__HIPCC__)
+#define DG_HD __host__ __device__
+#else
+#define DG_HD
+#endif
+
+namespace dgk {
+
+template <int NS> struct RK;
+template <> struct RK<5> {
+  DG_HD static constexpr double A(int s) {
+    return s == 0 ? 0.0
+         : s == 1 ? -567301805773.0 / 1357537059087.0
+         : s == 2 ? -2404267990393.0 / 2016746695238.0
+         : s == 3 ? -3550918686646.0 / 2091501179385.0
+                  : -1275806237668.0 / 842570457699.0;
+  }
+  DG_HD static constexpr double B(int s) {
+    return s == 0 ? 1432997174477.0 / 9575080441755.0
+         : s == 1 ? 5161836677717.0 / 13612068292357.0
+         : s == 2 ? 1720146321549.0 / 2090206949498.0
+         : s == 3 ? 3134564353537.0 / 4481467310338.0
+                  : 2277821191437.0 / 14882151754819.0;
+  }
+  DG_HD static constexpr double C(int s) {
+    return s == 0 ? 0.0
+         : s == 1 ? 1432997174477.0 / 9575080441755.0
+         : s == 2 ? 2526269341429.0 / 6820363962896.0
+         : s == 3 ? 2006345519317.0 / 3224310063776.0
+                  : 2802321613138.0 / 2924317926251.0;
+  }
+};
+template <> struct RK<1> {
+  DG_HD static constexpr double A(int) { return 0.0; }
+  DG_HD static constexpr double B(int) { return 1.0; }
+  DG_HD static constexpr double C(int) { return 0.0; }
+};
+
+struct RkPoly {
+  double beta[6];
+  double g[5][5];
+  double r[4];
+  bool ok;
+  long double lr[4];
+};
+
+inline const RkPoly& rk_poly() {
+  static const RkPoly P = [] {
+    long double uc[6] = {1}, rc[6] = {0}, uf[5][6] = {}, rf[5][6] = {};
+    for (int s = 0; s < 5; ++s) {
+      const long double A = RK<5>::A(s), B = RK<5>::B(s);
+      for (int k = 5; k >= 0; --k) rc[k] = A * rc[k] + (k ? uc[k - 1] : 0.0L);
+      for (int q = 0; q < 5; ++q)
+        for (int k = 5; k >= 0; --k)
+          rf[q][k] = A * rf[q][k] + (k ? uf[q][k - 1] : 0.0L) + ((q == s && k == 0) ? 1.0L : 0.0L);
+      for (int k = 0; k < 6; ++k) uc[k] += B * rc[k];
+      for (int q = 0; q < 5; ++q)
+        for (int k = 0; k < 6; ++k) uf[q][k] += B * rf[q][k];
+    }
+    RkPoly r{};
+    for (int k = 0; k < 6; ++k) r.beta[k] = double(uc[k]);
+    for (int q = 0; q < 5; ++q)
+      for (int k = 0; k < 5; ++k) r.g[q][k] = double(uf[q][k]);
+    r.ok = r.beta[0] == 1.0 && r.beta[1] == 1.0 && r.beta[2] != 0.0 && r.beta[3] != 0.0 &&
+           r.beta[4] != 0.0 && r.beta[5] != 0.0;
+    if (r.ok) {
+      r.lr[0] = uc[5] / uc[4];
+      r.lr[1] = uc[4] / uc[3];
+      r.lr[2] = uc[3] / uc[2];
+      r.lr[3] = uc[2];
+      for (int l = 0; l < 4; ++l) r.r[l] = double(r.lr[l]);
+    }
+    return r;
+  }();
+  return P;
+}
+
+constexpr bool horner_levels(int np) { return np != 3 && np <= 8; }
+constexpr int horner_blocks(int np) { return horner_levels(np) ? 5 : 1; }
+
+constexpr size_t kKernargMax = 4096;
+
+constexpr size_t eo_bytes(int np) { return 8u * size_t(2 * ((np + 1) / 2) * (np / 2) + np); }
+constexpr size_t rp_op_bytes(int np) { return size_t(horner_blocks(np)) * eo_bytes(np) + 8u * 9u; }
+constexpr size_t rp_step_args_bytes(int np, int ms) { return rp_op_bytes(np) + 8u * size_t(ms * 6 + 1) + 16u; }
+constexpr size_t rp_adj_args_bytes(int np) { return rp_op_bytes(np) + 16u; }
+constexpr size_t sweep_args_bytes(int np, int msf) {
+  return rp_op_bytes(np) + 8u * size_t((kSweepMaxSteps / msf) * (msf * 6 + 1)) +
+         8u * size_t(2 * (kSweepMaxSteps / 5 + 1) + 12) + 32u;
+}
+
+inline void horner_scale(const double* src, double* dst, int n, int level) {
+  const long double r = rk_poly().lr[level];
+  for (int i = 0; i < n; ++i) dst[i] = double(r * (long double)src[i]);
+}
+
+inline void horner_bnd(const double u[5], double bnd[5]) {
+  const RkPoly& P = rk_poly();
+  double b[5];
+  for (int k = 0; k < 5; ++k) {
+    double acc = 0.0;
+    for (int s = 0; s < 5; ++s) acc = std::fma(P.g[s][k], u[s], acc);
+    b[k] = acc;
+  }
+  bnd[0] = b[4] / P.beta[5];
+  for (int l = 1; l < 5; ++l) bnd[l] = b[4 - l];
+}
+
+}
diff --git a/adjoint-ode-adaptivity_amd/csrc/dg_ovl_tiles.h b/adjoint-ode-adaptivity_amd/csrc/dg_ovl_tiles.h
--- a/adjoint-ode-adaptivity_amd/csrc/dg_ovl_tiles.h
+++ b/adjoint-ode-adaptivity_amd/csrc/dg_ovl_tiles.h
@@ -137,7 +137,7 @@
                                              const double* __restrict__ uin,
                                              double* __restrict__ rec, double* __restrict__ last,
                                              const double* __restrict__ scale,
-                                             const RpOp<NP>& c, OpSrc<NP> os,
+                                             const RpOp<NP>& c, OpSrcF<NP> os,
                                              const double* kb, int64_t n0, bool jend) {
   using G = OvGeo<NP, NW>;
   constexpr int T = G::T, E = 2;
@@ -191,7 +191,7 @@
       const double fromL = ov_shr1(vN[E - 1]), fromR = ov_shl1(v0[0]);
       double pe[E][NE], po[E][NO];
       {
-        const auto& op = os.get();
+        const auto& op = os.un();
 #pragma unroll
         for (int m = 0; m < E; ++m) {
 #pragma unroll
@@ -242,7 +242,7 @@
         bnd = lds[CB + st * 5 + l];
         if (l == 0) urec = lds[CR + st];
       }
-      const auto& ol = os.get();
+      const auto& ol = os.un();
 #pragma unroll
       for (int m = 0; m < E; ++m) {
         double vL = (m == 0) ? fromL : vN[m - 1];
@@ -313,7 +313,7 @@
                                             const double* __restrict__ rec,
                                             EtaSink& es,
                                             const double* __restrict__ scale,
-                                            const RpOp<NP>& c, OpSrc<NP> os, int64_t n0) {
+                                            const RpOp<NP>& c, OpSrcA<NP, UNI> os, int64_t n0) {
   using G = OvGeo<NP, NW>;
   constexpr int T = G::T, E = 2;
   constexpr int H = RpHalo<MS>::A;
@@ -352,6 +352,7 @@
   }
   __syncthreads();
 
+  constexpr bool FOLD = kFold<NP, UNI>;
   const double b4 = c.beta[4], b5 = c.beta[5], b3 = c.beta[3], b2 = c.beta[2];
   double te[E][NE], to[E][NO];
 #pragma unroll 1
@@ -360,7 +361,7 @@
 #pragma unroll
     for (int m = 0; m <= E; ++m) jc[m] = jn[m];
     if (has_eta) {
-      const auto& op = os.get();
+      const auto& op = os.un();
 #pragma unroll
       for (int m = 0; m < E; ++m) {
         double pe = 0.0, po = 0.0;
@@ -380,7 +381,7 @@
 #pragma unroll
     for (int l = 0; l < 5; ++l) {
       double g0[E], g1[E], qe[E][NE], qo[E][NO];
-      const auto& ol = os.get();
+      const auto& ol = os.lv(l);
 #pragma unroll
       for (int m = 0; m < E; ++m) {
         double gd = 0.0, gs = 0.0;
@@ -401,14 +402,14 @@
       }
       const double fromL = ov_shr1(g1[E - 1]), fromR = ov_shl1(g0[0]);
       double ae[E][NE], ao[E][NO];
-      const auto& oq = os.get();
+      const auto& oq = os.lv(l);
 #pragma unroll
       for (int m = 0; m < E; ++m) {
 #pragma unroll
         for (int j = 0; j < NO; ++j) {
           double t;
           int k0 = 0;
-          if (l >= 3) {
+          if (FOLD || l >= 3) {
             t = wo[m][j];
           } else if (l >= 1) {
             t = (l == 1 ? b3 : b2) * wo[m][j];
@@ -424,7 +425,7 @@
         for (int j = 0; j < NE; ++j) {
           double t;
           int k0 = 0;
-          if (l >= 3) {
+          if (FOLD || l >= 3) {
             t = we[m][j];
           } else if (l >= 1) {
             t = (l == 1 ? b3 : b2) * we[m][j];
@@ -453,13 +454,13 @@
         ao[m][0] += gr - gl;
 #pragma unroll
         for (int k = 0; k < NE; ++k) {
-          if (l == 0) te[m][k] = fma(b5, ae[m][k], b4 * we[m][k]);
+          if (l == 0 && !FOLD) te[m][k] = fma(b5, ae[m][k], b4 * we[m][k]);
           else if (l < 4) te[m][k] = ae[m][k];
           else we[m][k] = ae[m][k];
         }
 #pragma unroll
         for (int k = 0; k < NO; ++k) {
-          if (l == 0) to[m][k] = fma(b5, ao[m][k], b4 * wo[m][k]);
+          if (l == 0 && !FOLD) to[m][k] = fma(b5, ao[m][k], b4 * wo[m][k]);
           else if (l < 4) to[m][k] = ao[m][k];
           else wo[m][k] = ao[m][k];
         }
diff --git a/adjoint-ode-adaptivity_amd/csrc/dg_rec.hip b/adjoint-ode-adaptivity_amd/csrc/dg_rec.hip
--- a/adjoint-ode-adaptivity_amd/csrc/dg_rec.hip
+++ b/adjoint-ode-adaptivity_amd/csrc/dg_rec.hip
@@ -10,12 +10,16 @@
   int64_t n0;
   int32_t jend;
 };
+static_assert(sizeof(RpStepArgs<8, 20>) == rp_step_args_bytes(8, 20) &&
+                  sizeof(RpStepArgs<9, 20>) == rp_step_args_bytes(9, 20),
+              "dg_horner.h's struct sizes");
 
 template <int NP, int MS> struct RpAdjArgs {
   RpOp<NP> c;
   int64_t n0;
   int32_t has_eta;
 };
+static_assert(sizeof(RpAdjArgs<8, 10>) == rp_adj_args_bytes(8), "dg_horner.h's struct sizes");
 
 template <int NP, bool UNI, int NW, int E, int MS>
 __global__ __launch_bounds__(64 * NW) void k_step_rp(const double* __restrict__ uin,
@@ -24,12 +28,14 @@
                                                         const double* __restrict__ scale,
                                                         RpStepArgs<NP, MS> args) {
   using G = RpGeo<NP, NW, E>;
+  static_assert(sizeof(RpStepArgs<NP, MS>) + 4 * sizeof(void*) <= kKernargMax,
+                "k_step_rp's arguments exceed the kernarg segment");
   __shared__ __attribute__((aligned(16))) double lds[G::kLds + MS * 6 + 1];
   const int64_t tile = tile_of(blockIdx.x, gridDim.x, args.c.xcd);
   constexpr int H = RpHalo<MS>::F;
   const int64_t e0 = tile * (G::T - 2 * H) - H;
   using SArgs = RpStepArgs<NP, MS>;
-  const OpSrc<NP> os = op_src<NP>(
+  const OpSrcF<NP> os = op_src<NP, false>(
       args.c, kernarg_tail_k<decltype(&k_step_rp<NP, UNI, NW, E, MS>), SArgs>() + offsetof(SArgs, c));
   if (edge_tile(e0, G::T, args.c.ktot, args.c.K)) {
     const double* kb = reinterpret_cast<const double*>(
@@ -50,13 +56,15 @@
                                                        const double* __restrict__ scale,
                                                        RpAdjArgs<NP, MS> args) {
   using G = RpGeo<NP, NW, E>;
+  static_assert(sizeof(RpAdjArgs<NP, MS>) + 5 * sizeof(void*) <= kKernargMax,
+                "k_adj_rp's arguments exceed the kernarg segment");
   __shared__ __attribute__((aligned(16))) double lds[G::kLds];
   const int64_t tile = tile_of(blockIdx.x, gridDim.x, args.c.xcd);
   constexpr int H = RpHalo<MS>::A;
   const int64_t e0 = tile * (G::T - 2 * H) - H;
   EtaSink es{eta, nullptr, nullptr, 0, 0, args.has_eta, false, 0.0, 0};
   using AArgs = RpAdjArgs<NP, MS>;
-  const OpSrc<NP> os = op_src<NP>(
+  const OpSrcA<NP, UNI> os = op_src<NP, kFold<NP, UNI>>(
       args.c, kernarg_tail_k<decltype(&k_adj_rp<NP, UNI, NW, E, MS>), AArgs>() + offsetof(AArgs, c));
   if (edge_tile(e0, G::T, args.c.ktot, args.c.K))
     rp_adj_tile<NP, UNI, NW, E, MS, true, false>(lds, tile, win, wout, rec, es, scale, args.c, os,
@@ -77,7 +85,7 @@
   constexpr int H = RpHalo<MS>::F;
   const int64_t e0 = tile * (G::T - 2 * H) - H;
   using SArgs = RpStepArgs<NP, MS>;
-  const OpSrc<NP> os = op_src<NP>(
+  const OpSrcF<NP> os = op_src<NP, false>(
       args.c, kernarg_tail_k<decltype(&k_step_rps<NP, UNI, NW, MS>), SArgs>() + offsetof(SArgs, c));
   const int64_t field = args.c.ktot * NP;
   double* last = snap + (MS - 1) * field;
diff --git a/adjoint-ode-adaptivity_amd/csrc/dg_rec_tiles.h b/adjoint-ode-adaptivity_amd/csrc/dg_rec_tiles.h
--- a/adjoint-ode-adaptivity_amd/csrc/dg_rec_tiles.h
+++ b/adjoint-ode-adaptivity_amd/csrc/dg_rec_tiles.h
@@ -214,64 +214,42 @@
   }
 }
 
-struct RkPoly {
-  double beta[6];
-  double g[5][5];
-  bool ok;
-};
-
-inline const RkPoly& rk_poly() {
-  static const RkPoly P = [] {
-    long double uc[6] = {1}, rc[6] = {0}, uf[5][6] = {}, rf[5][6] = {};
-    for (int s = 0; s < 5; ++s) {
-      const long double A = RK<5>::A(s), B = RK<5>::B(s);
-      for (int k = 5; k >= 0; --k) rc[k] = A * rc[k] + (k ? uc[k - 1] : 0.0L);
-      for (int q = 0; q < 5; ++q)
-        for (int k = 5; k >= 0; --k)
-          rf[q][k] = A * rf[q][k] + (k ? uf[q][k - 1] : 0.0L) + ((q == s && k == 0) ? 1.0L : 0.0L);
-      for (int k = 0; k < 6; ++k) uc[k] += B * rc[k];
-      for (int q = 0; q < 5; ++q)
-        for (int k = 0; k < 6; ++k) uf[q][k] += B * rf[q][k];
-    }
-    RkPoly r{};
-    for (int k = 0; k < 6; ++k) r.beta[k] = double(uc[k]);
-    for (int q = 0; q < 5; ++q)
-      for (int k = 0; k < 5; ++k) r.g[q][k] = double(uf[q][k]);
-    r.ok = r.beta[0] == 1.0 && r.beta[1] == 1.0 && r.beta[5] != 0.0;
-    return r;
-  }();
-  return P;
-}
+template <int NP, bool UNI> constexpr bool kFold = UNI && horner_levels(NP);
 
 inline void rp_block_bnd(const dg_plan* p, int MS, const double* times, double dt, double* bnd) {
-  const RkPoly& P = rk_poly();
   for (int m = 0; m < MS; ++m) {
-    double u[5], b[5];
+    double u[5];
     for (int s = 0; s < 5; ++s) u[s] = inflow_value(p, times[m] + RK<5>::C(s) * dt);
-    for (int k = 0; k < 5; ++k) {
-      double acc = 0.0;
-      for (int s = 0; s < 5; ++s) acc = std::fma(P.g[s][k], u[s], acc);
-      b[k] = acc;
-    }
-    bnd[m * 5 + 0] = b[4] / P.beta[5];
-    for (int l = 1; l < 5; ++l) bnd[m * 5 + l] = b[4 - l];
+    horner_bnd(u, bnd + m * 5);
   }
   for (int m = 0; m <= MS; ++m) bnd[MS * 5 + m] = inflow_value(p, times[m]);
 }
 
 template <int NP> struct RpOp {
-  EOArgs<NP> op;
+  static constexpr int NB = horner_blocks(NP), kUn = NB - 1;
+  EOArgs<NP> blk[NB];
   double sc;
   double beta[6];
   int64_t ktot;
   int32_t K;
   int32_t xcd;
 };
+static_assert(sizeof(EOArgs<2>) == eo_bytes(2) && sizeof(EOArgs<5>) == eo_bytes(5) &&
+                  sizeof(EOArgs<9>) == eo_bytes(9) && sizeof(RpOp<5>) == rp_op_bytes(5) &&
+                  sizeof(RpOp<8>) == rp_op_bytes(8) && sizeof(RpOp<9>) == rp_op_bytes(9),
+              "dg_horner.h's struct sizes");
 
 template <int NP> int rp_make_op(const dg_plan* p, double dt, RpOp<NP>* c) {
   const RkPoly& P = rk_poly();
-  if (!P.ok) return fail(DG_ERR_HIP, "LSERK4 stability polynomial: beta_0 = beta_1 = 1 expected");
-  make_eo<NP>(p, p->uniform ? dt * p->s_uniform : 1.0, &c->op, true);
+  if (!P.ok)
+    return fail(DG_ERR_HIP, "LSERK4 stability polynomial: beta_0 = beta_1 = 1 and nonzero "
+                            "beta_2 .. beta_5 expected");
+  using Op = RpOp<NP>;
+  make_eo<NP>(p, p->uniform ? dt * p->s_uniform : 1.0, &c->blk[Op::kUn], true);
+  static_assert(sizeof(EOArgs<NP>) % sizeof(double) == 0, "a block is an array of doubles");
+  for (int l = 0; l < Op::kUn; ++l)
+    horner_scale(reinterpret_cast<const double*>(&c->blk[Op::kUn]),
+                 reinterpret_cast<double*>(&c->blk[l]), int(sizeof(EOArgs<NP>) / sizeof(double)), l);
   c->sc = dt;
   for (int k = 0; k < 6; ++k) c->beta[k] = P.beta[k];
   c->ktot = p->ktot;
@@ -280,25 +258,32 @@
   return DG_OK;
 }
 
-template <int NP> constexpr bool kOpReload = NP >= 6;
-template <int NP, bool R = kOpReload<NP>> struct OpSrc {
+template <int NP, bool FOLDED> constexpr bool kOpReload = NP >= 6 || FOLDED;
+template <int NP, bool FOLDED, bool R = kOpReload<NP, FOLDED>> struct OpSrc {
   const EOArgs<NP>* p;
-  __device__ __forceinline__ const EOArgs<NP>& get() const { return *p; }
+  __device__ __forceinline__ const EOArgs<NP>& un() const { return p[RpOp<NP>::kUn]; }
+  __device__ __forceinline__ const EOArgs<NP>& lv(int) const { return un(); }
 };
-template <int NP> struct OpSrc<NP, true> {
+template <int NP, bool FOLDED> struct OpSrc<NP, FOLDED, true> {
   const DG_KAS EOArgs<NP>* p;
-  __device__ __forceinline__ const DG_KAS EOArgs<NP>& get() const {
-    const DG_KAS EOArgs<NP>* q = p;
+  __device__ __forceinline__ const DG_KAS EOArgs<NP>& at(int i) const {
+    const DG_KAS EOArgs<NP>* q = p + i;
     asm volatile("" : "+s"(q));
     return *q;
   }
+  __device__ __forceinline__ const DG_KAS EOArgs<NP>& un() const { return at(RpOp<NP>::kUn); }
+  __device__ __forceinline__ const DG_KAS EOArgs<NP>& lv(int l) const {
+    return at(FOLDED ? l : RpOp<NP>::kUn);
+  }
 };
-template <int NP>
-__device__ __forceinline__ OpSrc<NP> op_src(const RpOp<NP>& rc, const DG_KAS char* kc) {
-  if constexpr (kOpReload<NP>)
-    return OpSrc<NP>{reinterpret_cast<const DG_KAS EOArgs<NP>*>(kc + offsetof(RpOp<NP>, op))};
+template <int NP> using OpSrcF = OpSrc<NP, false>;
+template <int NP, bool UNI> using OpSrcA = OpSrc<NP, kFold<NP, UNI>>;
+template <int NP, bool FOLDED>
+__device__ __forceinline__ OpSrc<NP, FOLDED> op_src(const RpOp<NP>& rc, const DG_KAS char* kc) {
+  if constexpr (kOpReload<NP, FOLDED>)
+    return OpSrc<NP, FOLDED>{reinterpret_cast<const DG_KAS EOArgs<NP>*>(kc + offsetof(RpOp<NP>, blk))};
   else
-    return OpSrc<NP>{&rc.op};
+    return OpSrc<NP, FOLDED>{rc.blk};
 }
 
 template <int NP, int E, bool EDGE>
@@ -330,7 +315,7 @@
                                              const double* __restrict__ uin,
                                              double* __restrict__ rec, double* __restrict__ last,
                                              const double* __restrict__ scale,
-                                             const RpOp<NP>& c, OpSrc<NP> os,
+                                             const RpOp<NP>& c, OpSrcF<NP> os,
                                              const double* kb, int64_t n0, bool jend,
                                              int64_t sstride = 0) {
   static_assert(!SNAP || (E == 2 && !WT), "snapshots: launch chains on pair tiles");
@@ -391,7 +376,7 @@
       __builtin_amdgcn_sched_barrier(0);
       double pe[E][NE], po[E][NO];
       {
-        const auto& op = os.get();
+        const auto& op = os.un();
 #pragma unroll
         for (int m = 0; m < E; ++m) {
 #pragma unroll
@@ -414,7 +399,7 @@
         }
       }
       {
-        const auto& op = os.get();
+        const auto& op = os.un();
 #pragma unroll
         for (int m = 0; m < E; ++m) {
 #pragma unroll
@@ -450,7 +435,7 @@
         bnd = lds[CB + st * 5 + l];
         if (l == 0) urec = lds[CR + st];
       }
-      const auto& ol = os.get();
+      const auto& ol = os.un();
 #pragma unroll
       for (int m = 0; m < E; ++m) {
         double vL = (m == 0) ? fromL : vN[m - 1];
@@ -546,7 +531,7 @@
                                             const double* __restrict__ rec,
                                             EtaSink& es,
                                             const double* __restrict__ scale,
-                                            const RpOp<NP>& c, OpSrc<NP> os, int64_t n0) {
+                                            const RpOp<NP>& c, OpSrcA<NP, UNI> os, int64_t n0) {
   using G = RpGeo<NP, NW, E>;
   constexpr int T = G::T, LB = G::LB;
   constexpr int H = RpHalo<MS>::A;
@@ -586,6 +571,7 @@
   }
   __syncthreads();
 
+  constexpr bool FOLD = kFold<NP, UNI>;
   const double b4 = c.beta[4], b5 = c.beta[5], b3 = c.beta[3], b2 = c.beta[2];
   double te[E][NE], to[E][NO];
 #pragma unroll 1
@@ -594,7 +580,7 @@
 #pragma unroll
     for (int m = 0; m <= E; ++m) jc[m] = jn[m];
     if (has_eta) {
-      const auto& op = os.get();
+      const auto& op = os.un();
 #pragma unroll
       for (int m = 0; m < E; ++m) {
         double pe = 0.0, po = 0.0;
@@ -615,7 +601,7 @@
     for (int l = 0; l < 5; ++l) {
       const int f0 = (((MS - 1 - st) * 5 + l) & 1) * 2 * FB, f1 = f0 + FB;
       double g0[E], g1[E], qe[E][NE], qo[E][NO];
-      const auto& ol = os.get();
+      const auto& ol = os.lv(l);
 #pragma unroll
       for (int m = 0; m < E; ++m) {
         double gd = 0.0, gs = 0.0;
@@ -638,14 +624,14 @@
       lds[f1 + lane + 1] = g1[E - 1];
       __builtin_amdgcn_sched_barrier(0);
       double ae[E][NE], ao[E][NO];
-      const auto& oq = os.get();
+      const auto& oq = os.lv(l);
 #pragma unroll
       for (int m = 0; m < E; ++m) {
 #pragma unroll
         for (int j = 0; j < NO; ++j) {
           double t;
           int k0 = 0;
-          if (l >= 3) {
+          if (FOLD || l >= 3) {
             t = wo[m][j];
           } else if (l >= 1) {
             t = (l == 1 ? b3 : b2) * wo[m][j];
@@ -661,14 +647,14 @@
         for (int k = 0; k < NO; ++k) pin(ao[m][k]);
       }
       __builtin_amdgcn_sched_barrier(0);
-      const auto& or_ = os.get();
+      const auto& or_ = os.lv(l);
 #pragma unroll
       for (int m = 0; m < E; ++m) {
 #pragma unroll
         for (int j = 0; j < NE; ++j) {
           double t;
           int k0 = 0;
-          if (l >= 3) {
+          if (FOLD || l >= 3) {
             t = we[m][j];
           } else if (l >= 1) {
             t = (l == 1 ? b3 : b2) * we[m][j];
@@ -697,13 +683,13 @@
         ao[m][0] += gr - gl;
 #pragma unroll
         for (int k = 0; k < NE; ++k) {
-          if (l == 0) te[m][k] = fma(b5, ae[m][k], b4 * we[m][k]);
+          if (l == 0 && !FOLD) te[m][k] = fma(b5, ae[m][k], b4 * we[m][k]);
           else if (l < 4) te[m][k] = ae[m][k];
           else we[m][k] = ae[m][k];
         }
 #pragma unroll
         for (int k = 0; k < NO; ++k) {
-          if (l == 0) to[m][k] = fma(b5, ao[m][k], b4 * wo[m][k]);
+          if (l == 0 && !FOLD) to[m][k] = fma(b5, ao[m][k], b4 * wo[m][k]);
           else if (l < 4) to[m][k] = ao[m][k];
           else wo[m][k] = ao[m][k];
         }
diff --git a/adjoint-ode-adaptivity_amd/csrc/dg_sweep_kernel.h b/adjoint-ode-adaptivity_amd/csrc/dg_sweep_kernel.h
--- a/adjoint-ode-adaptivity_amd/csrc/dg_sweep_kernel.h
+++ b/adjoint-ode-adaptivity_amd/csrc/dg_sweep_kernel.h
@@ -28,6 +28,10 @@
   int32_t mode;
   int32_t spin_limit;
 };
+static_assert(sizeof(SweepArgs<5, 20>) == sweep_args_bytes(5, 20) &&
+                  sizeof(SweepArgs<8, 5>) == sweep_args_bytes(8, 5) &&
+                  sizeof(SweepArgs<9, 5>) == sweep_args_bytes(9, 5),
+              "dg_horner.h's struct sizes");
 
 template <int NP, bool UNI, int NW = 8, int X = 0> struct SweepOcc {
   static constexpr int waves_per_simd =
@@ -109,7 +113,8 @@
     const uint64_t t_ready = a.trace ? uint64_t(wall_clock64()) : 0;
     using SA = SweepArgs<NP, MSF>;
     const DG_KAS char* ka = kernarg_tail_k<decltype(&k_sweep_rp<NP, UNI, NW, MSF, MSA, E, X>), SA>();
-    const OpSrc<NP> os = op_src<NP>(a.c, ka + offsetof(SA, c));
+    const OpSrcF<NP> osf = op_src<NP, false>(a.c, ka + offsetof(SA, c));
+    const OpSrcA<NP, UNI> osa = op_src<NP, kFold<NP, UNI>>(a.c, ka + offsetof(SA, c));
     if (fwd) {
       const int64_t e0 = int64_t(j) * TEF - HF;
       const double* kb = reinterpret_cast<const double*>(
@@ -120,17 +125,17 @@
       if constexpr (X == 1) {
         if (edge_tile(e0, G::T, ktot, a.c.K))
           ov_step_tile<NP, UNI, NW, MSF, true, true>(lds, j, a.U[blk], a.rec, a.U[blk + 1],
-                                                     a.scale, a.c, os, kb, n0, jend);
+                                                     a.scale, a.c, osf, kb, n0, jend);
         else
           ov_step_tile<NP, UNI, NW, MSF, false, true>(lds, j, a.U[blk], a.rec, a.U[blk + 1],
-                                                      a.scale, a.c, os, kb, n0, jend);
+                                                      a.scale, a.c, osf, kb, n0, jend);
       } else {
         if (edge_tile(e0, G::T, ktot, a.c.K))
           rp_step_tile<NP, UNI, NW, E, MSF, true, true>(lds, j, a.U[blk], a.rec, a.U[blk + 1],
-                                                        a.scale, a.c, os, kb, n0, jend);
+                                                        a.scale, a.c, osf, kb, n0, jend);
         else
           rp_step_tile<NP, UNI, NW, E, MSF, false, true>(lds, j, a.U[blk], a.rec, a.U[blk + 1],
-                                                         a.scale, a.c, os, kb, n0, jend);
+                                                         a.scale, a.c, osf, kb, n0, jend);
       }
       if (s_bad) {
         asm volatile("s_waitcnt vmcnt(0)" ::: "memory");
@@ -160,17 +165,17 @@
       if constexpr (X == 1) {
         if (edge_tile(e0, G::T, ktot, a.c.K))
           ov_adj_tile<NP, UNI, NW, MSA, true, true>(lds, j, a.W[blk], a.W[blk + 1], a.rec, es,
-                                                    a.scale, a.c, os, n0);
+                                                    a.scale, a.c, osa, n0);
         else
           ov_adj_tile<NP, UNI, NW, MSA, false, true>(lds, j, a.W[blk], a.W[blk + 1], a.rec, es,
-                                                     a.scale, a.c, os, n0);
+                                                     a.scale, a.c, osa, n0);
       } else {
         if (edge_tile(e0, G::T, ktot, a.c.K))
           rp_adj_tile<NP, UNI, NW, E, MSA, true, true>(lds, j, a.W[blk], a.W[blk + 1], a.rec, es,
-                                                       a.scale, a.c, os, n0);
+                                                       a.scale, a.c, osa, n0);
         else
           rp_adj_tile<NP, UNI, NW, E, MSA, false, true>(lds, j, a.W[blk], a.W[blk + 1], a.rec,
-                                                        es, a.scale, a.c, os, n0);
+                                                        es, a.scale, a.c, osa, n0);
       }
       if (s_bad) {
         asm volatile("s_waitcnt vmcnt(0)" ::: "memory");
diff --git a/profiles/horner_levels/summarize.py b/profiles/horner_levels/summarize.py
--- /dev/null
+++ b/profiles/horner_levels/summarize.py
@@ -0,0 +1,28 @@
+import glob
+import json
+import os
+import statistics
+
+HERE = os.path.dirname(os.path.abspath(__file__))
+ARGS = {"N4": "", "N1": "--N 1", "N2": "--N 2", "N6": "--N 6", "K65536": "--K 65536 --ics 1024"}
+out = {}
+for shape, args in ARGS.items():
+  row = {"bench_arguments": args}
+  for who in ("parent", "new"):
+    files = sorted(glob.glob(os.path.join(HERE, "runs", f"ab_{shape}_{who}_*.json")))
+    runs = [json.load(open(f)) for f in files]
+    ms = [r["ms_per_step"] for r in runs]
+    row[who] = {"ms_per_step": ms, "median": statistics.median(ms), "min": min(ms), "max": max(ms),
+                "value_median": statistics.median(r["value"] for r in runs)}
+  row["new_median_over_parent_median"] = row["new"]["median"] / row["parent"]["median"]
+  row["gain"] = row["new"]["median"] < row["parent"]["min"]
+  out[shape] = row
+for who in ("parent", "new"):
+  out[f"pmc_{who}"] = json.load(open(os.path.join(HERE, f"pmc_{who}.json")))["per_launch"]
+json.dump(out, open(os.path.join(HERE, "summary.json"), "w"), indent=1)
+for shape in ARGS:
+  r = out[shape]
+  print(f"{shape}: parent {r['parent']['median']:.5f} [{r['parent']['min']:.5f}, {r['parent']['max']:.5f}]  "
+        f"new {r['new']['median']:.5f} [{r['new']['min']:.5f}, {r['new']['max']:.5f}]  "
+        f"ratio {r['new_median_over_parent_median']:.4f}  gain {r['gain']}  "
+        f"value {r['parent']['value_median']:.4g} -> {r['new']['value_median']:.4g}")
```

Result: faster. 828.5 billion (median of 6 runs) (+1.9%).
